# mengcaopku/DCNet

Hardware: AMD Instinct MI355X
Metric: clips/sec (T=8, 416x416, bs8) fwd+bwd (higher is better)
Workload: dtype f32; 1 GPU; T=8 416x416 bs8/GPU L=20 fp32, 64 img/GPU/step as pairs, fwd+5 losses+bwd+RMSprop; arith=f16x2-split MFMA, fp32 accumulate, parallelism=dp1, ranks_seen=1, reducer=none, step=hipGraph replay (fwd+losses+bwd+RMSprop), sampler=mt

## Files before the change

### dcnet_amd/csrc/coattn.hip

```cpp
#include "igemm.h"
#include "prof.h"
#include "coattn.h"

int tn_gemm_batched(const float* A, int lda, long long a_bs, const float* B, int ldb, long long b_bs,
                    float* C, int ldc, long long c_bs, const float* row_scale,
                    int M, int m_ld, int N, int K, int batch, int accumulate, hipStream_t stream,
                    const unsigned* amax_a = nullptr, const unsigned* amax_b = nullptr);

namespace {

constexpr int EXP_ROWS = 32;

typedef _Float16 f16x4c_t __attribute__((ext_vector_type(4)));
constexpr float E_SPLIT_SCALE = 8192.f;
template <bool SPLIT>
__global__ __launch_bounds__(256) void exp_sums_kernel(float* __restrict__ E, int hw, int ldE, float t,
                                                       float* __restrict__ rsum, float* __restrict__ colpart) {
  __shared__ float red[4][EXP_ROWS];
  const int b = blockIdx.y, rb = blockIdx.x;
  const int i0 = rb * EXP_ROWS;
  float* e = E + ((size_t)b * hw + i0) * ldE;
  float racc[EXP_ROWS];
#pragma unroll
  for (int r = 0; r < EXP_ROWS; ++r) racc[r] = 0.f;
  const int nrow = min(EXP_ROWS, hw - i0);
  for (int j = threadIdx.x * 4; j < ldE; j += 1024) {
    f32x4 v[EXP_ROWS];
#pragma unroll
    for (int r = 0; r < EXP_ROWS; ++r)
      v[r] = r < nrow ? *reinterpret_cast<const f32x4*>(e + (size_t)r * ldE + j) : f32x4{0.f, 0.f, 0.f, 0.f};
    f32x4 cs = {0.f, 0.f, 0.f, 0.f};
#pragma unroll
    for (int r = 0; r < EXP_ROWS; ++r) {
      if (r < nrow) {
        f32x4 o;
#pragma unroll
        for (int k = 0; k < 4; ++k) o[k] = (j + k < hw) ? expf(t * v[r][k] - t) : 0.f;
        if constexpr (SPLIT) {
          const f32x4 ts = o * E_SPLIT_SCALE;
          const f16x4c_t h = {(_Float16)ts[0], (_Float16)ts[1], (_Float16)ts[2], (_Float16)ts[3]};
          const f16x4c_t l = {(_Float16)(ts[0] - (float)h[0]), (_Float16)(ts[1] - (float)h[1]), (_Float16)(ts[2] - (float)h[2]),
                              (_Float16)(ts[3] - (float)h[3])};
          unsigned char* run = reinterpret_cast<unsigned char*>(e + (size_t)r * ldE + (j & ~7)) + (j & 4) * 2;
          *reinterpret_cast<f16x4c_t*>(run) = h;
          *reinterpret_cast<f16x4c_t*>(run + 16) = l;
        } else {
          *reinterpret_cast<f32x4*>(e + (size_t)r * ldE + j) = o;
        }
        cs += o; racc[r] += (o[0] + o[1]) + (o[2] + o[3]);
      }
    }
    *reinterpret_cast<f32x4*>(colpart + ((size_t)rb * gridDim.y + b) * ldE + j) = cs;
  }
  const int lane = threadIdx.x & 63, wave = threadIdx.x >> 6;
#pragma unroll
  for (int r = 0; r < EXP_ROWS; ++r) {
    const float s = wave_sum(racc[r]);
    if (lane == 0) red[wave][r] = s;
  }
  __syncthreads();
  if (threadIdx.x < EXP_ROWS && i0 + threadIdx.x < hw)
    rsum[(size_t)b * hw + i0 + threadIdx.x] = 1.f / (red[0][threadIdx.x] + red[1][threadIdx.x] + red[2][threadIdx.x] + red[3][threadIdx.x]);
}

__global__ __launch_bounds__(256) void colsum_inv_kernel(const float* __restrict__ colpart, int nrb, int b, int hw, int ldE,
                                                         float* __restrict__ cinv) {
  const int j = blockIdx.x * 256 + threadIdx.x, bb = blockIdx.y;
  if (j >= hw) return;
  float s = 0.f;
  for (int rb = 0; rb < nrb; ++rb) s += colpart[((size_t)rb * b + bb) * ldE + j];
  cinv[(size_t)bb * hw + j] = 1.f / s;
}

enum { AM_ONE = 0, AM_DO1, AM_DO2, AM_DO1S, AM_DO2S, AM_DA, AM_DP1, AM_DP2, AM_SLOTS };
__global__ __launch_bounds__(256) void amax_init_kernel(unsigned* __restrict__ w) {
  for (int i = threadIdx.x; i < AM_SLOTS * DCN_AMAX_WORDS; i += 256) w[i] = i < DCN_AMAX_WORDS ? 0x3F800000u : 0u;
}

__global__ __launch_bounds__(256) void rowdot_scale_kernel(const float* __restrict__ d, int ldd, int64_t bsd,
                                                           const float* __restrict__ o, int ldo, int64_t bso, int hw,
                                                           const float* __restrict__ inv, int64_t rows, int c,
                                                           float* __restrict__ delta, float* __restrict__ ds,
                                                           unsigned* __restrict__ amax_d, unsigned* __restrict__ amax_ds) {
  __shared__ float red[4];
  const int lane = threadIdx.x & 63;
  const int64_t row = (int64_t)blockIdx.x * 4 + (threadIdx.x >> 6);
  float vmax = 0.f, s = 0.f;
  if (row < rows) {
    const int64_t bb = row / hw, i = row - bb * hw;
    s = inv[row];
    float acc = 0.f;
    for (int k = lane * 4; k < c; k += 256) {
      const f32x4 dv = *reinterpret_cast<const f32x4*>(d + bb * bsd + i * ldd + k);
      const f32x4 ov = *reinterpret_cast<const f32x4*>(o + bb * bso + i * ldo + k);
      acc += dv[0] * ov[0] + dv[1] * ov[1] + dv[2] * ov[2] + dv[3] * ov[3];
      *reinterpret_cast<f32x4*>(ds + row * c + k) = dv * s;
      vmax = fmaxf(fmaxf(vmax, fmaxf(fabsf(dv[0]), fabsf(dv[1]))), fmaxf(fabsf(dv[2]), fabsf(dv[3])));
    }
    acc = wave_sum(acc);
    if (lane == 0) delta[row] = acc;
  }
  const float vs = wave_max(vmax * s);
  amax_update_block(amax_d, vmax, red);
  __syncthreads();
  amax_update_block(amax_ds, vs, red);
}

template <bool ESPLIT, bool OSPLIT = false>
__global__ __launch_bounds__(256) void dA_kernel(const float* __restrict__ E, float* __restrict__ dP1, const float* __restrict__ dP2,
                                                 const float* __restrict__ rinv, const float* __restrict__ cinv,
                                                 const float* __restrict__ d1, const float* __restrict__ d2,
                                                 int hw, int ldE, float t, int64_t total4, unsigned* __restrict__ amax_da) {
  __shared__ float red[4];
  float vmax = 0.f;
  const int l4 = ldE >> 2;
  float s_out = 1.f;
  if constexpr (OSPLIT) {
    const int be = (int)((amax_read(amax_da) >> 23) & 0xFF);
    int ex = (be == 0 || be == 255) ? 0 : 14 - (be - 126);
    ex = ex > 100 ? 100 : (ex < -100 ? -100 : ex);
    s_out = __uint_as_float((unsigned)(ex + 127) << 23);
  }
  for (int64_t idx = (int64_t)blockIdx.x * 256 + threadIdx.x; idx < total4; idx += (int64_t)gridDim.x * 256) {
    const int64_t row = idx / l4;
    const int j = (int)(idx - row * l4) * 4;
    const int64_t bb = row / hw;
    f32x4 e;
    if constexpr (ESPLIT) {
      const unsigned char* run = reinterpret_cast<const unsigned char*>(E + row * ldE + (j & ~7)) + (j & 4) * 2;
      const f16x4c_t h = *reinterpret_cast<const f16x4c_t*>(run), l = *reinterpret_cast<const f16x4c_t*>(run + 16);
#pragma unroll
      for (int k = 0; k < 4; ++k) e[k] = ((float)h[k] + (float)l[k]) * (1.f / E_SPLIT_SCALE);
    } else {
      e = *reinterpret_cast<const f32x4*>(E + row * ldE + j);
    }
    const f32x4 p1 = *reinterpret_cast<const f32x4*>(dP1 + row * ldE + j);
    const f32x4 p2 = *reinterpret_cast<const f32x4*>(dP2 + row * ldE + j);
    const float ri = rinv[row], di = d1[row];
    f32x4 o;
#pragma unroll
    for (int k = 0; k < 4; ++k) {
      float v = 0.f;
      if (j + k < hw) v = t * e[k] * ((p1[k] - di) * ri + (p2[k] - d2[bb * hw + j + k]) * cinv[bb * hw + j + k]);
      o[k] = v;
    }
    if constexpr (OSPLIT) {
      const f32x4 ts = o * s_out;
      const f16x4c_t h = {(_Float16)ts[0], (_Float16)ts[1], (_Float16)ts[2], (_Float16)ts[3]};
      const f16x4c_t l = {(_Float16)(ts[0] - (float)h[0]), (_Float16)(ts[1] - (float)h[1]), (_Float16)(ts[2] - (float)h[2]),
                          (_Float16)(ts[3] - (float)h[3])};
      unsigned char* run = reinterpret_cast<unsigned char*>(dP1 + row * ldE + (j & ~7)) + (j & 4) * 2;
      *reinterpret_cast<f16x4c_t*>(run) = h;
      *reinterpret_cast<f16x4c_t*>(run + 16) = l;
    } else {
      *reinterpret_cast<f32x4*>(dP1 + row * ldE + j) = o;
      vmax = fmaxf(fmaxf(vmax, fmaxf(fabsf(o[0]), fabsf(o[1]))), fmaxf(fabsf(o[2]), fabsf(o[3])));
    }
  }
  if constexpr (!OSPLIT) amax_update_block(amax_da, vmax, red);
}

__global__ __launch_bounds__(64) void da_bound_kernel(const unsigned* __restrict__ a1, const unsigned* __restrict__ a2, float t,
                                                      unsigned* __restrict__ out) {
  const float b = 2.f * t * (__uint_as_float(amax_read(a1)) + __uint_as_float(amax_read(a2)));
  out[threadIdx.x & (DCN_AMAX_WORDS - 1)] = __float_as_uint(b);
}

inline int ld_pad(int hw) { return (hw + 31) / 32 * 32; }

void gemm_params(IgemmParams& p, const float* A, int lda, long long a_bs, const float* B, int ldb, long long b_bs,
                 float* C, int ldc, long long c_bs, int M, int N, int K, int batch) {
  p = IgemmParams{};
  p.osy = p.osx = p.isy = p.isx = 1; p.dense_out = 1;
  p.in = A; p.ldi = lda; p.in_bs = a_bs; p.wt = B; p.ldw = ldb; p.wt_bs = b_bs; p.out = C; p.ldo = ldc; p.out_bs = c_bs;
  p.ldr = ldc;
  p.N = 1; p.Hi = 1; p.Wi = M; p.Ho = 1; p.Wo = M; p.Hs = 1; p.Ws = M; p.M = M;
  p.Ci = K; p.Co = N; p.ntaps = 1; p.batch = batch;
}

}

static bool on_gemm3(int b, int hw, int c) { return c % 32 == 0 && gemm3_applicable(hw, c, hw, b) && gemm3_applicable(hw, hw, c, b); }

int coattn_ld_pad(int hw) { return ld_pad(hw); }
bool coattn_on_gemm3(int b, int hw, int c) { return on_gemm3(b, hw, c); }
unsigned* coattn_ws_amax(float* ws, int b, int hw) { return reinterpret_cast<unsigned*>(ws + (int64_t)cdiv(hw, EXP_ROWS) * b * ld_pad(hw)); }
int coattn_amax_init(unsigned* am, hipStream_t stream) {
  hipLaunchKernelGGL(amax_init_kernel, dim3(1), dim3(256), 0, stream, am);
  DCN_CHECK_LAUNCH("coattn amax_init");
  return DCN_OK;
}
int coattn_exp_sums(float* E, int b, int hw, float temperature, float* rinv, float* cinv, float* ws, bool split, hipStream_t stream) {
  const int ldE = ld_pad(hw), nrb = cdiv(hw, EXP_ROWS);
  const int pid = prof_begin(12, (double)b * hw * ldE * 8.0, stream);
  if (split) hipLaunchKernelGGL(exp_sums_kernel<true>, dim3(nrb, b), dim3(256), 0, stream, E, hw, ldE, temperature, rinv, ws);
  else hipLaunchKernelGGL(exp_sums_kernel<false>, dim3(nrb, b), dim3(256), 0, stream, E, hw, ldE, temperature, rinv, ws);
  prof_end(pid, stream);
  DCN_CHECK_LAUNCH("exp_sums");
  hipLaunchKernelGGL(colsum_inv_kernel, dim3(cdiv(hw, 256), b), dim3(256), 0, stream, ws, nrb, b, hw, ldE, cinv);
  DCN_CHECK_LAUNCH("colsum_inv");
  return DCN_OK;
}

extern "C" int64_t dcn_coattn_fwd_ws(int b, int hw, int c) {
  (void)c;
  return (int64_t)cdiv(hw, EXP_ROWS) * b * ld_pad(hw) + AM_SLOTS * DCN_AMAX_WORDS;
}
extern "C" int64_t dcn_coattn_e_size(int b, int hw) { return (int64_t)b * hw * ld_pad(hw); }
extern "C" int64_t dcn_coattn_saved_size(int b, int hw, int c) {
  return dcn_coattn_e_size(b, hw) + (on_gemm3(b, hw, c) ? (int64_t)2 * b * hw * c : 0);
}

extern "C" int dcn_coattn_fwd(const float* f1, const float* f2, int ldf, int64_t bsf, float* f1_attn, float* f2_attn, int ldo,
                              int64_t bso, float* E, float* rinv, float* cinv, float* ws,
                              int b, int hw, int c, float temperature, void* stream_) {
  hipStream_t stream = (hipStream_t)stream_;
  DCN_CHECK_ARG(f1 && f2 && f1_attn && E && rinv && cinv && ws, "coattn_fwd: null pointer");
  DCN_CHECK_ARG(b > 0 && hw > 0 && c > 0 && c % 32 == 0, "coattn_fwd: bad shape (c=%d must be a multiple of 32)", c);
  if (ldf <= 0) ldf = c;
  if (ldo <= 0) ldo = c;
  DCN_CHECK_ARG(ldf % 4 == 0 && ldo % 4 == 0, "coattn_fwd: ldf/ldo must be multiples of 4");
  if (bsf <= 0) bsf = (int64_t)hw * ldf;
  if (bso <= 0) bso = (int64_t)hw * ldo;
  DCN_CHECK_ARG(bsf % 4 == 0 && bso % 4 == 0, "coattn_fwd: batch strides must be multiples of 4");
  const int ldE = ld_pad(hw);
  unsigned* am = reinterpret_cast<unsigned*>(ws + (int64_t)cdiv(hw, EXP_ROWS) * b * ldE);
  hipLaunchKernelGGL(amax_init_kernel, dim3(1), dim3(256), 0, stream, am);
  DCN_CHECK_LAUNCH("coattn amax_init");
  const unsigned* one = am + AM_ONE * DCN_AMAX_WORDS;
  const int nrb = cdiv(hw, EXP_ROWS);
  const long long bsE = (long long)hw * ldE;
  if (on_gemm3(b, hw, c)) {
    float* f1s = E + dcn_coattn_e_size(b, hw);
    float* f2s = f1s + (int64_t)b * hw * c;
    const long long bss = (long long)hw * c;
    int rc = gemm3_presplit(f1, ldf, bsf, f1s, c, bss, b, hw, c, one, stream);
    if (rc) return rc;
    if ((rc = gemm3_presplit(f2, ldf, bsf, f2s, c, bss, b, hw, c, one, stream))) return rc;
    if ((rc = gemm3_launch(f1s, c, bss, 0, f2s, c, bss, 0, E, ldE, bsE, nullptr, 0, hw, hw, c, b, 0, one, one, stream))) return rc;
    const int pid = prof_begin(12, (double)b * hw * ldE * 8.0, stream);
    hipLaunchKernelGGL(exp_sums_kernel<true>, dim3(nrb, b), dim3(256), 0, stream, E, hw, ldE, temperature, rinv, ws);
    prof_end(pid, stream);
    DCN_CHECK_LAUNCH("exp_sums");
    hipLaunchKernelGGL(colsum_inv_kernel, dim3(cdiv(hw, 256), b), dim3(256), 0, stream, ws, nrb, b, hw, ldE, cinv);
    DCN_CHECK_LAUNCH("colsum_inv");
    if ((rc = gemm3_launch(E, ldE, bsE, 0, f2s, c, bss, 1, f1_attn, ldo, bso, rinv, hw, hw, c, hw, b, 0, one, one, stream))) return rc;
    if (f2_attn) rc = gemm3_launch(E, ldE, bsE, 1, f1s, c, bss, 1, f2_attn, ldo, bso, cinv, hw, hw, c, hw, b, 0, one, one, stream);
    return rc;
  }
  IgemmParams p;
  gemm_params(p, f1, ldf, bsf, f2, ldf, bsf, E, ldE, (long long)hw * ldE, hw, hw, c, b);
  p.amax_a = one; p.amax_b = one;
  int rc = igemm_launch(p, stream);
  if (rc) return rc;
  const int pid = prof_begin(12, (double)b * hw * ldE * 8.0, stream);
  hipLaunchKernelGGL(exp_sums_kernel<false>, dim3(nrb, b), dim3(256), 0, stream, E, hw, ldE, temperature, rinv, ws);
  prof_end(pid, stream);
  DCN_CHECK_LAUNCH("exp_sums");
  hipLaunchKernelGGL(colsum_inv_kernel, dim3(cdiv(hw, 256), b), dim3(256), 0, stream, ws, nrb, b, hw, ldE, cinv);
  DCN_CHECK_LAUNCH("colsum_inv");
  gemm_params(p, E, ldE, (long long)hw * ldE, f2, ldf, bsf, f1_attn, ldo, bso, hw, c, ldE, b);
  p.bmode = 1; p.kvalid = hw; p.row_scale = rinv; p.amax_a = one; p.amax_b = one;
  rc = igemm_launch(p, stream);
  if (rc) return rc;
  if (f2_attn)
    rc = tn_gemm_batched(E, ldE, (long long)hw * ldE, f1, ldf, bsf, f2_attn, ldo, bso,
                         cinv, hw, ldE, c, hw, b, 0, stream, one, one);
  return rc;
}

extern "C" int64_t dcn_coattn_bwd_ws(int b, int hw, int c) {
  return (int64_t)2 * b * hw * ld_pad(hw) + (int64_t)2 * b * hw * c + (int64_t)2 * b * hw + AM_SLOTS * DCN_AMAX_WORDS +
         (on_gemm3(b, hw, c) ? (int64_t)2 * b * hw * c + 4 : 0);
}

extern "C" int dcn_coattn_bwd(const float* f1, const float* f2, int ldf, int64_t bsf,
                              const float* d_f1_attn, const float* d_f2_attn, int lddo, int64_t bsdo,
                              const float* f1_attn, const float* f2_attn, int ldo, int64_t bso,
                              const float* E, const float* rinv, const float* cinv,
                              float* d_f1, float* d_f2, int lddf, int64_t bsdf, int accumulate, float* ws,
                              int b, int hw, int c, float temperature, void* stream_) {
  hipStream_t stream = (hipStream_t)stream_;
  DCN_CHECK_ARG(f1 && f2 && d_f1_attn && d_f2_attn && f1_attn && f2_attn && E && rinv && cinv && d_f1 && d_f2 && ws,
                "coattn_bwd: null pointer");
  DCN_CHECK_ARG(b > 0 && hw > 0 && c > 0 && c % 32 == 0, "coattn_bwd: bad shape");
  if (ldf <= 0) ldf = c;
  if (ldo <= 0) ldo = c;
  if (lddo <= 0) lddo = c;
  if (lddf <= 0) lddf = c;
  if (bsf <= 0) bsf = (int64_t)hw * ldf;
  if (bso <= 0) bso = (int64_t)hw * ldo;
  if (bsdo <= 0) bsdo = (int64_t)hw * lddo;
  if (bsdf <= 0) bsdf = (int64_t)hw * lddf;
  const int ldE = ld_pad(hw);
  const long long rows = (long long)b * hw;
  float* dP1 = ws;
  float* dP2 = dP1 + rows * ldE;
  float* dO1s = dP2 + rows * ldE;
  float* dO2s = dO1s + rows * c;
  float* del1 = dO2s + rows * c;
  float* del2 = del1 + rows;
  unsigned* am = reinterpret_cast<unsigned*>(del2 + rows);
  hipLaunchKernelGGL(amax_init_kernel, dim3(1), dim3(256), 0, stream, am);
  DCN_CHECK_LAUNCH("coattn amax_init");
  auto slot = [&](int i) { return am + i * DCN_AMAX_WORDS; };
  hipLaunchKernelGGL(rowdot_scale_kernel, dim3(cdiv(rows, 4)), dim3(256), 0, stream, d_f1_attn, lddo, bsdo, f1_attn, ldo, bso, hw, rinv, rows, c, del1, dO1s,
                     slot(AM_DO1), slot(AM_DO1S));
  DCN_CHECK_LAUNCH("rowdot_scale");
  hipLaunchKernelGGL(rowdot_scale_kernel, dim3(cdiv(rows, 4)), dim3(256), 0, stream, d_f2_attn, lddo, bsdo, f2_attn, ldo, bso, hw, cinv, rows, c, del2, dO2s,
                     slot(AM_DO2), slot(AM_DO2S));
  DCN_CHECK_LAUNCH("rowdot_scale");
  const int64_t total4 = rows * (ldE / 4);
  int64_t g = (total4 + 255) / 256; if (g > 8192) g = 8192;
  if (g > 1024) g = 1024;
  const long long bsE = (long long)hw * ldE;
  if (on_gemm3(b, hw, c)) {
    float* dO1p = reinterpret_cast<float*>(((uintptr_t)(am + AM_SLOTS * DCN_AMAX_WORDS) + 15) & ~(uintptr_t)15);
    float* dO2p = dO1p + rows * c;
    const float* f1s = E + dcn_coattn_e_size(b, hw);
    const float* f2s = f1s + rows * c;
    const long long bss = (long long)hw * c;
    int rc;
    if ((rc = gemm3_presplit(d_f1_attn, lddo, bsdo, dO1p, c, bss, b, hw, c, slot(AM_DO1), stream))) return rc;
    if ((rc = gemm3_presplit(d_f2_attn, lddo, bsdo, dO2p, c, bss, b, hw, c, slot(AM_DO2), stream))) return rc;
    if ((rc = gemm3_presplit(dO1s, c, bss, dO1s, c, bss, b, hw, c, slot(AM_DO1S), stream))) return rc;
    if ((rc = gemm3_presplit(dO2s, c, bss, dO2s, c, bss, b, hw, c, slot(AM_DO2S), stream))) return rc;
    if ((rc = gemm3_launch(dO1p, c, bss, 0, f2s, c, bss, 0, dP1, ldE, bsE, nullptr, 0, hw, hw, c, b, 0, slot(AM_DO1), slot(AM_ONE), stream, slot(AM_DP1)))) return rc;
    if ((rc = gemm3_launch(f1s, c, bss, 0, dO2p, c, bss, 0, dP2, ldE, bsE, nullptr, 0, hw, hw, c, b, 0, slot(AM_ONE), slot(AM_DO2), stream, slot(AM_DP2)))) return rc;
    hipLaunchKernelGGL(da_bound_kernel, dim3(1), dim3(64), 0, stream, slot(AM_DP1), slot(AM_DP2), temperature, slot(AM_DA));
    DCN_CHECK_LAUNCH("dA bound");
    const int pid_da = prof_begin(31, (double)total4 * 16.0 * 4.0, stream);
    hipLaunchKernelGGL((dA_kernel<true, true>), dim3((int)g), dim3(256), 0, stream, E, dP1, dP2, rinv, cinv, del1, del2, hw, ldE, temperature, total4, slot(AM_DA));
    prof_end(pid_da, stream);
    DCN_CHECK_LAUNCH("dA");
    if ((rc = gemm3_launch(dP1, ldE, bsE, 0, f2s, c, bss, 1, d_f1, lddf, bsdf, nullptr, 0, hw, c, hw, b, accumulate, slot(AM_DA), slot(AM_ONE), stream))) return rc;
    if ((rc = gemm3_launch(E, ldE, bsE, 0, dO2s, c, bss, 1, d_f1, lddf, bsdf, nullptr, 0, hw, c, hw, b, 1, slot(AM_ONE), slot(AM_DO2S), stream))) return rc;
    if ((rc = gemm3_launch(dP1, ldE, bsE, 1, f1s, c, bss, 1, d_f2, lddf, bsdf, nullptr, 0, hw, c, hw, b, accumulate, slot(AM_DA), slot(AM_ONE), stream))) return rc;
    return gemm3_launch(E, ldE, bsE, 1, dO1s, c, bss, 1, d_f2, lddf, bsdf, nullptr, 0, hw, c, hw, b, 1, slot(AM_ONE), slot(AM_DO1S), stream);
  }
  IgemmParams p;
  int rc;
  gemm_params(p, d_f1_attn, lddo, bsdo, f2, ldf, bsf, dP1, ldE, (long long)hw * ldE, hw, hw, c, b);
  p.amax_a = slot(AM_DO1); p.amax_b = slot(AM_ONE);
  if ((rc = igemm_launch(p, stream))) return rc;
  gemm_params(p, f1, ldf, bsf, d_f2_attn, lddo, bsdo, dP2, ldE, (long long)hw * ldE, hw, hw, c, b);
  p.amax_a = slot(AM_ONE); p.amax_b = slot(AM_DO2);
  if ((rc = igemm_launch(p, stream))) return rc;
  const int pid_da = prof_begin(31, (double)total4 * 16.0 * 4.0, stream);
  hipLaunchKernelGGL(dA_kernel<false>, dim3((int)g), dim3(256), 0, stream, E, dP1, dP2, rinv, cinv, del1, del2, hw, ldE, temperature, total4, slot(AM_DA));
  prof_end(pid_da, stream);
  DCN_CHECK_LAUNCH("dA");
  gemm_params(p, dP1, ldE, (long long)hw * ldE, f2, ldf, bsf, d_f1, lddf, bsdf, hw, c, ldE, b);
  p.bmode = 1; p.kvalid = hw; p.accumulate = accumulate; p.amax_a = slot(AM_DA); p.amax_b = slot(AM_ONE);
  if ((rc = igemm_launch(p, stream))) return rc;
  gemm_params(p, E, ldE, (long long)hw * ldE, dO2s, c, (long long)hw * c, d_f1, lddf, bsdf, hw, c, ldE, b);
  p.bmode = 1; p.kvalid = hw; p.accumulate = 1; p.amax_a = slot(AM_ONE); p.amax_b = slot(AM_DO2S);
  if ((rc = igemm_launch(p, stream))) return rc;
  rc = tn_gemm_batched(dP1, ldE, (long long)hw * ldE, f1, ldf, bsf, d_f2, lddf, bsdf,
                       nullptr, hw, ldE, c, hw, b, accumulate, stream, slot(AM_DA), slot(AM_ONE));
  if (rc) return rc;
  return tn_gemm_batched(E, ldE, (long long)hw * ldE, dO1s, c, (long long)hw * c, d_f2, lddf, bsdf,
                         nullptr, hw, ldE, c, hw, b, 1, stream, slot(AM_ONE), slot(AM_DO1S));
}
```

### dcnet_amd/csrc/gemm3.hip

```cpp
#include "igemm.h"
#include "prof.h"

namespace {

typedef _Float16 f16x8_t __attribute__((ext_vector_type(8)));
typedef short s16x4 __attribute__((ext_vector_type(4)));
typedef short s16x8 __attribute__((ext_vector_type(8)));
typedef __attribute__((address_space(3))) void lds_void;

#ifndef G3_ABL
#define G3_ABL 0
#endif
constexpr unsigned G3_OOB = 0x80000000u;
constexpr int G3_BM = 256, G3_BN = 256, G3_STAGES = 4;
constexpr int G3_TILE = 256 * 64;
constexpr int G3_STAGE = 2 * G3_TILE;
constexpr int G3_LDS = G3_STAGES * G3_STAGE;

__device__ __forceinline__ float g3_pow2_scale(unsigned amax_bits) {
  const int be = (int)((amax_bits >> 23) & 0xFF);
  if (be == 0 || be == 255) return 1.f;
  int e = 14 - (be - 126);
  e = e > 100 ? 100 : (e < -100 ? -100 : e);
  return __uint_as_float((unsigned)(e + 127) << 23);
}

struct G3Params {
  const float* A; const float* B; float* C;
  long long a_bs, b_bs, c_bs;
  int lda, ldb, ldc;
  int M, N, K;
  int a_rows, b_rows;
  int a_cols, b_cols;
  int tiles_m, tiles_n;
  const float* row_scale; long long rs_bs;
  int accumulate;
  const unsigned* amax_a; const unsigned* amax_b;
  unsigned* amax_out;
  int var;
  int abl;
};

__device__ __forceinline__ int g3_tswz(int krow) { return (krow & 1) | ((krow & 2) << 1); }

template <bool AT, bool BT, bool H1 = false>
__global__ __launch_bounds__(512, 1) void gemm3_kernel(const G3Params p) {
  extern __shared__ __attribute__((aligned(1024))) unsigned char smem3g[];
  const int tid = threadIdx.x, lane = tid & 63;
  const int wave = __builtin_amdgcn_readfirstlane(tid >> 6);
  const int wm = wave >> 2, wn = wave & 3;
  const int per_batch = p.tiles_m * p.tiles_n;
  const int lin = xcd_remap(blockIdx.x, gridDim.x);
  const int batch = __builtin_amdgcn_readfirstlane(lin / per_batch), t_ = lin - batch * per_batch;
  const int bm = __builtin_amdgcn_readfirstlane(t_ / p.tiles_n), bn = t_ - bm * p.tiles_n;
  const int m0 = bm * G3_BM, n0 = bn * G3_BN;
  const int kslices = (p.K + 15) >> 4;

  const float* a_base = p.A + batch * p.a_bs + (AT ? 0 : (long long)m0 * p.lda);
  const float* b_base = p.B + batch * p.b_bs + (BT ? 0 : (long long)n0 * p.ldb);
  const int a_rows_left = AT ? p.a_rows : p.a_rows - m0, b_rows_left = BT ? p.b_rows : p.b_rows - n0;
  const long long a_bytes = ((long long)(a_rows_left - 1) * p.lda + p.a_cols) * 4, b_bytes = ((long long)(b_rows_left - 1) * p.ldb + p.b_cols) * 4;
  const __amdgpu_buffer_rsrc_t a_rs = __builtin_amdgcn_make_buffer_rsrc((void*)a_base, 0, a_bytes > 0x7FFFFFF0LL ? 0x7FFFFFF0 : (int)a_bytes, 0x00020000);
  const __amdgpu_buffer_rsrc_t b_rs = __builtin_amdgcn_make_buffer_rsrc((void*)b_base, 0, b_bytes > 0x7FFFFFF0LL ? 0x7FFFFFF0 : (int)b_bytes, 0x00020000);

  unsigned voff[4];
  int sstep_a, sstep_b;
#pragma unroll
  for (int e = 0; e < 2; ++e) {
    const int j = 2 * wave + e;
    if (AT) {
      voff[e] = (unsigned)((long long)j * p.lda * 4 + m0 * 4 + ((lane ^ g3_tswz(j)) << 4));
      if (m0 + ((lane ^ g3_tswz(j)) << 2) >= p.a_cols) voff[e] = G3_OOB;
    } else {
      const int row = 16 * j + (lane >> 2), c = (lane & 3) ^ ((row >> 2) & 3);
      voff[e] = row < a_rows_left ? (unsigned)((long long)row * p.lda * 4 + c * 16) : G3_OOB;
    }
    if (BT) {
      voff[2 + e] = (unsigned)((long long)j * p.ldb * 4 + n0 * 4 + ((lane ^ g3_tswz(j)) << 4));
      if (n0 + ((lane ^ g3_tswz(j)) << 2) >= p.b_cols) voff[2 + e] = G3_OOB;
    } else {
      const int row = 16 * j + (lane >> 2), c = (lane & 3) ^ ((row >> 2) & 3);
      voff[2 + e] = row < b_rows_left ? (unsigned)((long long)row * p.ldb * 4 + c * 16) : G3_OOB;
    }
  }
  sstep_a = AT ? 16 * p.lda * 4 : 64;
  sstep_b = BT ? 16 * p.ldb * 4 : 64;
  const int my_dst = 2 * wave * 1024;

  int k_done = 0;
  auto issue_a = [&]() {
    const bool live = k_done < kslices && !(G3_ABL && (p.abl & 1));
    unsigned char* st = smem3g + (k_done & (G3_STAGES - 1)) * G3_STAGE + my_dst;
    int sa_ = live ? k_done * sstep_a : 0;
    if (G3_ABL && (p.abl & 8)) sa_ = 0;
#pragma unroll
    for (int e = 0; e < 2; ++e)
      __builtin_amdgcn_raw_ptr_buffer_load_lds(a_rs, (lds_void*)(st + e * 1024), 16, (int)(live ? voff[e] : G3_OOB), sa_, 0, 0);
  };
  auto issue_b = [&]() {
    const bool live = k_done < kslices && !(G3_ABL && (p.abl & 1));
    unsigned char* st = smem3g + (k_done & (G3_STAGES - 1)) * G3_STAGE + my_dst;
    int sb_ = live ? k_done * sstep_b : 0;
    if (G3_ABL && (p.abl & 8)) sb_ = 0;
#pragma unroll
    for (int e = 0; e < 2; ++e)
      __builtin_amdgcn_raw_ptr_buffer_load_lds(b_rs, (lds_void*)(st + G3_TILE + e * 1024), 16, (int)(live ? voff[2 + e] : G3_OOB), sb_, 0, 0);
    ++k_done;
  };
  auto issue = [&]() { issue_a(); issue_b(); };

  const int g = lane >> 5;
  const int hh = lane >> 5, gg = (lane >> 4) & 1, qq = (lane & 15) >> 2, pp = lane & 3;
  int a_rd[4][2], b_rd[2][2];
#pragma unroll
  for (int mi = 0; mi < 4; ++mi) {
    if (AT) {
      const int c = wm * 128 + mi * 32 + 16 * gg + 4 * pp;
#pragma unroll
      for (int r2 = 0; r2 < 2; ++r2) {
        const int kr = 8 * hh + 4 * r2 + qq;
        a_rd[mi][r2] = kr * 1024 + ((((c >> 3) * 2) ^ g3_tswz(kr)) << 4) + (c & 7) * 2;
      }
    } else {
      const int ar = wm * 128 + mi * 32 + (lane & 31);
      a_rd[mi][0] = ar * 64 + (((2 * g) ^ ((ar >> 2) & 3)) << 4);
      a_rd[mi][1] = ar * 64 + (((2 * g + 1) ^ ((ar >> 2) & 3)) << 4);
    }
  }
#pragma unroll
  for (int ni = 0; ni < 2; ++ni) {
    if (BT) {
      const int c = wn * 64 + ni * 32 + 16 * gg + 4 * pp;
#pragma unroll
      for (int r2 = 0; r2 < 2; ++r2) {
        const int kr = 8 * hh + 4 * r2 + qq;
        b_rd[ni][r2] = G3_TILE + kr * 1024 + ((((c >> 3) * 2) ^ g3_tswz(kr)) << 4) + (c & 7) * 2;
      }
    } else {
      const int br = wn * 64 + ni * 32 + (lane & 31);
      b_rd[ni][0] = G3_TILE + br * 64 + (((2 * g) ^ ((br >> 2) & 3)) << 4);
      b_rd[ni][1] = G3_TILE + br * 64 + (((2 * g + 1) ^ ((br >> 2) & 3)) << 4);
    }
  }
  auto tr_read = [&](const unsigned char* ptr) {
    return __builtin_amdgcn_ds_read_tr16_b64_v4i16((__attribute__((address_space(3))) s16x4*)(ptr));
  };
  auto tfrag = [&](const unsigned char* st, int off0, int off1, int plane) {
    const s16x4 lo = tr_read(st + (off0 ^ (plane << 4))), hi = tr_read(st + (off1 ^ (plane << 4)));
    const s16x8 v = {lo[0], lo[1], lo[2], lo[3], hi[0], hi[1], hi[2], hi[3]};
    return __builtin_bit_cast(f16x8_t, v);
  };

  f32x16 acc[4][2];
#pragma unroll
  for (int mi = 0; mi < 4; ++mi)
#pragma unroll
    for (int ni = 0; ni < 2; ++ni)
#pragma unroll
      for (int r = 0; r < 16; ++r) acc[mi][ni][r] = 0.f;

  for (int s = 0; s < G3_STAGES - 1; ++s) issue();

  asm volatile("s_waitcnt vmcnt(%0)" :: "n"((G3_STAGES - 2) * 4) : "memory");
  if (wm == 1) __builtin_amdgcn_s_barrier();
  for (int it = 0; it < kslices; ++it) {
    __builtin_amdgcn_s_barrier();
    asm volatile("" ::: "memory");
    const unsigned char* st = smem3g + (it & (G3_STAGES - 1)) * G3_STAGE;
    f16x8_t bh[2], bl[2];
    f16x8_t ah[4], al[4];
    if (G3_ABL && (p.abl & 2)) {
#pragma unroll
      for (int ni = 0; ni < 2; ++ni) { bh[ni] = f16x8_t{(_Float16)it, 0, 0, 0, 0, 0, 0, 0}; bl[ni] = bh[ni]; }
#pragma unroll
      for (int mi = 0; mi < 4; ++mi) { ah[mi] = bh[0]; al[mi] = bh[1]; }
    } else {
#pragma unroll
      for (int ni = 0; ni < 2; ++ni) {
        if (BT) { bh[ni] = tfrag(st, b_rd[ni][0], b_rd[ni][1], 0); if constexpr (!H1) bl[ni] = tfrag(st, b_rd[ni][0], b_rd[ni][1], 1); }
        else { bh[ni] = *reinterpret_cast<const f16x8_t*>(st + b_rd[ni][0]); if constexpr (!H1) bl[ni] = *reinterpret_cast<const f16x8_t*>(st + b_rd[ni][1]); }
      }
#pragma unroll
      for (int mi = 0; mi < 4; ++mi) {
        if (AT) { ah[mi] = tfrag(st, a_rd[mi][0], a_rd[mi][1], 0); if constexpr (!H1) al[mi] = tfrag(st, a_rd[mi][0], a_rd[mi][1], 1); }
        else { ah[mi] = *reinterpret_cast<const f16x8_t*>(st + a_rd[mi][0]); if constexpr (!H1) al[mi] = *reinterpret_cast<const f16x8_t*>(st + a_rd[mi][1]); }
      }
    }
    if (p.var >= 1) {
      issue_a();
      if (wm == 1) asm volatile("s_waitcnt vmcnt(%0)" :: "n"((G3_STAGES - 2) * 4 - 2) : "memory");
    } else {
      issue();
      if (wm == 1) asm volatile("s_waitcnt vmcnt(%0)" :: "n"((G3_STAGES - 2) * 4) : "memory");
    }
    asm volatile("s_waitcnt lgkmcnt(0)" ::: "memory");
    __builtin_amdgcn_s_barrier();
    asm volatile("" ::: "memory");
    if (G3_ABL && (p.abl & 4)) {
#pragma unroll
      for (int mi = 0; mi < 4; ++mi) { asm volatile("" :: "v"(ah[mi]), "v"(al[mi])); }
#pragma unroll
      for (int ni = 0; ni < 2; ++ni) { asm volatile("" :: "v"(bh[ni]), "v"(bl[ni])); }
    } else {
      __builtin_amdgcn_s_setprio(1);
      if constexpr (!H1) {
#pragma unroll
        for (int mi = 0; mi < 4; ++mi)
#pragma unroll
          for (int ni = 0; ni < 2; ++ni) acc[mi][ni] = __builtin_amdgcn_mfma_f32_32x32x16_f16(al[mi], bh[ni], acc[mi][ni], 0, 0, 0);
        if (p.var == 2) issue_b();
#pragma unroll
        for (int mi = 0; mi < 4; ++mi)
#pragma unroll
          for (int ni = 0; ni < 2; ++ni) acc[mi][ni] = __builtin_amdgcn_mfma_f32_32x32x16_f16(ah[mi], bl[ni], acc[mi][ni], 0, 0, 0);
      } else if (p.var == 2) issue_b();
#pragma unroll
      for (int mi = 0; mi < 4; ++mi)
#pragma unroll
        for (int ni = 0; ni < 2; ++ni) acc[mi][ni] = __builtin_amdgcn_mfma_f32_32x32x16_f16(ah[mi], bh[ni], acc[mi][ni], 0, 0, 0);
      __builtin_amdgcn_s_setprio(0);
    }
    if (p.var == 1) issue_b();
    if (wm == 0) asm volatile("s_waitcnt vmcnt(%0)" :: "n"((G3_STAGES - 2) * 4) : "memory");
  }
  if (wm == 0) __builtin_amdgcn_s_barrier();
  asm volatile("s_waitcnt vmcnt(0)" ::: "memory");

  const float dq = 1.f / (g3_pow2_scale(amax_read(p.amax_a)) * g3_pow2_scale(amax_read(p.amax_b)));
  float* __restrict__ cb = p.C + batch * p.c_bs;
  const float* rs = p.row_scale ? p.row_scale + batch * p.rs_bs : nullptr;
  float vmax = 0.f;
#pragma unroll
  for (int mi = 0; mi < 4; ++mi)
#pragma unroll
    for (int r = 0; r < 16; ++r) {
      const int m = m0 + wm * 128 + mi * 32 + 4 * g + (r & 3) + 8 * (r >> 2);
      if (m >= p.M) continue;
      const float f = rs ? dq * rs[m] : dq;
#pragma unroll
      for (int ni = 0; ni < 2; ++ni) {
        const int n = n0 + wn * 64 + ni * 32 + (lane & 31);
        if (n >= p.N) continue;
        float v = acc[mi][ni][r] * f;
        float* dst = cb + (long long)m * p.ldc + n;
        if (p.accumulate) v += *dst;
        *dst = v;
        vmax = fmaxf(vmax, fabsf(v));
      }
    }
  if (p.amax_out) {
    vmax = wave_max(vmax);
    if (lane == 0) amax_update(p.amax_out, vmax, blockIdx.x * 8 + wave);
  }
}

__global__ __launch_bounds__(256) void presplit_kernel(const float* __restrict__ src, int ld, long long bs, float* __restrict__ dst, int ldd,
                                                        long long bsd, int rows, int c, long long total8, const unsigned* __restrict__ amax) {
  const float s = g3_pow2_scale(amax_read(amax));
  const int c8 = c >> 3;
  for (long long i = (long long)blockIdx.x * 256 + threadIdx.x; i < total8; i += (long long)gridDim.x * 256) {
    const long long row_all = i / c8; const int o = (int)(i - row_all * c8);
    const long long b = row_all / rows; const int row = (int)(row_all - b * rows);
    const float* sp = src + b * bs + (long long)row * ld + o * 8;
    const f32x4 x0 = *reinterpret_cast<const f32x4*>(sp) * s, x1 = *reinterpret_cast<const f32x4*>(sp + 4) * s;
    f16x8_t h, l;
#pragma unroll
    for (int e = 0; e < 4; ++e) { h[e] = (_Float16)x0[e]; h[4 + e] = (_Float16)x1[e]; }
#pragma unroll
    for (int e = 0; e < 4; ++e) { l[e] = (_Float16)(x0[e] - (float)h[e]); l[4 + e] = (_Float16)(x1[e] - (float)h[4 + e]); }
    float* dp = dst + b * bsd + (long long)row * ldd + o * 8;
    *reinterpret_cast<f16x8_t*>(dp) = h;
    *reinterpret_cast<f16x8_t*>(dp + 4) = l;
  }
}

DCN_KNOB(g_gemm3, "Gemm3", 1, "gemm3.hip: the co-attention products on pre-split operands (0 = implicit-GEMM / weight-gradient tiles; + 256 * v = schedule variant v; + 16 * bits = timing ablations, results WRONG)",
         nullptr, "-DG3_ABL=1", G3_ABL != 0, [](int v) { return (v & 0xF0) != 0; });
DCN_KNOB(g_gemm3_h1, "H1gemm3", 1, "gemm3.hip: one f16 piece per operand in the bf16 precision modes (0 = both pieces, fp32-accurate co-attention)");

template <bool AT, bool BT, bool H1>
int launch3g_(const G3Params& p, int grid, hipStream_t stream) {
  static DcnPerDeviceFlag attr_once;
  if (attr_once.first()) {
    (void)hipFuncSetAttribute(reinterpret_cast<const void*>(&gemm3_kernel<AT, BT, H1>), hipFuncAttributeMaxDynamicSharedMemorySize, G3_LDS);
  }
  hipLaunchKernelGGL((gemm3_kernel<AT, BT, H1>), dim3(grid), dim3(512), G3_LDS, stream, p);
  return DCN_OK;
}
template <bool AT, bool BT>
int launch3g(const G3Params& p, int grid, hipStream_t stream) {
  if (g_gemm3_h1 && igemm_precision() == 2) return launch3g_<AT, BT, true>(p, grid, stream);
  return launch3g_<AT, BT, false>(p, grid, stream);
}

}

int gemm3_variant() { const int v = g_gemm3 >> 8; return (v == 1 || v == 2) ? v : 0; }
extern "C" int dcn_gemm3_variant() { return gemm3_variant(); }

bool gemm3_applicable(int M, int N, int K, int batch) {
  return g_gemm3 && (igemm_precision() == 4 || igemm_precision() == 2) && M >= 512 && N >= 256 && K >= 64 && batch >= 1;
}

int gemm3_presplit(const float* src, int ld, long long bs, float* dst, int ldd, long long bsd, int batch, int rows, int c,
                   const unsigned* amax, hipStream_t stream) {
  DCN_CHECK_ARG(src && dst && amax && c % 8 == 0 && ld % 4 == 0 && ldd % 4 == 0 && bs % 4 == 0 && bsd % 4 == 0, "gemm3_presplit: bad argument");
  const long long total8 = (long long)batch * rows * (c / 8);
  long long g = (total8 + 255) / 256; if (g > 16384) g = 16384;
  hipLaunchKernelGGL(presplit_kernel, dim3((int)g), dim3(256), 0, stream, src, ld, bs, dst, ldd, bsd, rows, c, total8, amax);
  DCN_CHECK_LAUNCH("gemm3_presplit");
  return DCN_OK;
}

int gemm3_launch(const float* A, int lda, long long a_bs, int at, const float* B, int ldb, long long b_bs, int bt,
                 float* C, int ldc, long long c_bs, const float* row_scale, long long rs_bs,
                 int M, int N, int K, int batch, int accumulate, const unsigned* amax_a, const unsigned* amax_b, hipStream_t stream,
                 unsigned* amax_out) {
  DCN_CHECK_ARG(A && B && C && amax_a && amax_b, "gemm3: null pointer");
  DCN_CHECK_ARG(lda % 4 == 0 && ldb % 4 == 0 && a_bs % 4 == 0 && b_bs % 4 == 0 && (((uintptr_t)A | (uintptr_t)B) & 15) == 0, "gemm3: 16-byte rows");
  G3Params p{};
  p.A = A; p.B = B; p.C = C; p.a_bs = a_bs; p.b_bs = b_bs; p.c_bs = c_bs; p.lda = lda; p.ldb = ldb; p.ldc = ldc;
  p.M = M; p.N = N; p.K = K;
  const int k16 = (K + 15) / 16 * 16;
  p.a_rows = at ? K : M; p.b_rows = bt ? K : N;
  p.a_cols = at ? (M + 7) / 8 * 8 : k16; p.b_cols = bt ? (N + 7) / 8 * 8 : k16;
  DCN_CHECK_ARG(p.a_cols <= lda && p.b_cols <= ldb, "gemm3: rows shorter than the tile reads (lda=%d ldb=%d)", lda, ldb);
  p.tiles_m = cdiv(M, G3_BM); p.tiles_n = cdiv(N, G3_BN);
  p.row_scale = row_scale; p.rs_bs = rs_bs; p.accumulate = accumulate; p.amax_a = amax_a; p.amax_b = amax_b; p.amax_out = amax_out; p.abl = (g_gemm3 >> 4) & 15; p.var = gemm3_variant();
  const int grid = p.tiles_m * p.tiles_n * batch;
  const int pid = prof_begin(40, 2.0 * batch * (double)M * N * K, stream);
  int rc;
  if (at) rc = bt ? launch3g<true, true>(p, grid, stream) : DCN_ERR_ARG;
  else rc = bt ? launch3g<false, true>(p, grid, stream) : launch3g<false, false>(p, grid, stream);
  prof_end(pid, stream);
  DCN_CHECK_ARG(rc == DCN_OK, "gemm3: no A^T . B^T form");
  DCN_CHECK_LAUNCH("gemm3");
  return DCN_OK;
}

extern "C" int dcn_gemm3_supported(int m, int n, int k, int batch) { return gemm3_applicable(m, n, k, batch) ? 1 : 0; }

extern "C" int dcn_gemm3_presplit(const float* src, int ld, int64_t bs, float* dst, int ldd, int64_t bsd, int batch, int rows, int c,
                                  const uint32_t* amax, void* stream) {
  return gemm3_presplit(src, ld, bs, dst, ldd, bsd, batch, rows, c, amax, (hipStream_t)stream);
}

extern "C" int dcn_gemm3(const float* a, int lda, int64_t a_bs, int a_t, const float* b, int ldb, int64_t b_bs, int b_t,
                         float* c, int ldc, int64_t c_bs, const float* row_scale, int64_t rs_bs,
                         int m, int n, int k, int batch, int accumulate, const uint32_t* amax_a, const uint32_t* amax_b, void* stream) {
  DCN_CHECK_ARG(m > 0 && n > 0 && k > 0 && batch > 0, "gemm3: empty problem");
  return gemm3_launch(a, lda, a_bs, a_t, b, ldb, b_bs, b_t, c, ldc, c_bs, row_scale, rs_bs, m, n, k, batch, accumulate, amax_a, amax_b,
                      (hipStream_t)stream, nullptr);
}
```

### dcnet_amd/csrc/igemm.h

```cpp
#pragma once
#include "common.h"

#define IGEMM_MAX_TAPS 16


struct IgemmParams {
  const float* in;
  const float* wt;
  const float* f8;
  const unsigned* amax_a;
  const unsigned* amax_b;
  const void* wt16;
  const float* b_scale;
  unsigned* amax_out;
  float* out;
  const float* scale;
  const float* shift;
  const float* residual;
  float* stats;
  const float* row_scale;
  int batch;
  long long in_bs, wt_bs, out_bs;
  int bmode;
  int kvalid;
  int N, Hi, Wi, Ci, ldi;
  int Ho, Wo;
  int Hs, Ws;
  int oy0, ox0, osy, osx;
  int isy, isx;
  int Co, ldo, ldr, ldw;
  int M;
  int ntaps;
  int cpt, kiters;
  int act; float slope;
  int accumulate, dense_out, c4;
  int tap_dy[IGEMM_MAX_TAPS], tap_dx[IGEMM_MAX_TAPS], tap_w[IGEMM_MAX_TAPS];
  int ncls;
  int cls_M[4], cls_Hs[4], cls_Ws[4], cls_oy0[4], cls_ox0[4], cls_ntaps[4];
  const float* bt_y; const float* bt_mean; const float* bt_invstd; const float* bt_gamma; const float* bt_beta;
  int bt_act; float bt_slope;
  const unsigned char* a_scale8; const unsigned char* b_scale8;
};
inline double epilogue_reads(const IgemmParams& p) { return 1.0 + (p.accumulate ? 1.0 : 0.0) + (p.residual ? 1.0 : 0.0) + (p.bt_y ? 1.0 : 0.0); }
bool igemm_tap_capable(const IgemmParams& p);

int igemm_grid_m(int M, int Co, int ntaps);
int igemm_launch(const IgemmParams& p, hipStream_t stream);
bool igemm_will_presplit(long long rows, int Co, int ntaps, int Ci);

bool conv3_applicable(const IgemmParams& p, int precision, int gran);
int conv3_launch(const IgemmParams& p, int gran, hipStream_t stream);
bool conv3x_takes(const IgemmParams& p, int gran);
int conv3x_launch(const IgemmParams& p, int gran, hipStream_t stream);
int conv3b_bm(int M, int Co, int Wi);
bool conv3b_takes(const IgemmParams& p);
int conv3b_launch(const IgemmParams& p, int out_f32, hipStream_t stream);

bool conv1_applicable(const IgemmParams& p, int precision, int gran);
int conv1_launch(const IgemmParams& p, int gran, hipStream_t stream);
int conv1_tile_of(long long rows, int Co, int ntaps, int Ci, int stats, int gran, int storage16);
int conv1b_grid_m(int M, int Co, int ntaps, int s1_w = 0);
int conv1b_launch(const IgemmParams& p, int out_f32, hipStream_t stream);
int conv1q_grid_m(int M, int Co);
int conv1q_launch(const IgemmParams& p, int out_f32, hipStream_t stream);
bool conv2b_takes(int M, int Co, int ntaps);
int conv2b_launch(const IgemmParams& p, int out_f32, hipStream_t stream);


bool stem_applicable(const IgemmParams& p, const float* scratch);
int stem_launch(const IgemmParams& p, float* scratch, hipStream_t stream);

bool dgrad2_applicable(int n, int h, int wd, int cin, int cout, int ksize, int stride, int accumulate);
struct DcnBnTap { const float* y; const float* mean; const float* invstd; const float* gamma; const float* beta; int act; float slope;
                  float* stats; int stats_rows; };
int nconv1_launch_b16(int mode, const void* x, int ldi, const void* w16, void* y, int ldo, float* stats, int stats_rows,
                      int n, int h, int wd, int stride, hipStream_t stream);
int dgrad2_launch_b16(const void* dy, int lddy, const void* wt16, void* dx, int n, int h, int wd, int cin, int accumulate, hipStream_t stream);
int dgrad2_grid(int n, int h, int wd, int cin);
int dgrad2_launch(const float* dy, int lddy, const float* wt, float* dx, int n, int h, int wd, int cin, int accumulate,
                  const uint32_t* amax_dy, const uint32_t* amax_w, const DcnBnTap* tap, hipStream_t stream);
bool gemm3_applicable(int M, int N, int K, int batch);
int gemm3_presplit(const float* src, int ld, long long bs, float* dst, int ldd, long long bsd, int batch, int rows, int c,
                   const unsigned* amax, hipStream_t stream);
int gemm3_launch(const float* A, int lda, long long a_bs, int at, const float* B, int ldb, long long b_bs, int bt,
                 float* C, int ldc, long long c_bs, const float* row_scale, long long rs_bs,
                 int M, int N, int K, int batch, int accumulate, const unsigned* amax_a, const unsigned* amax_b, hipStream_t stream,
                 unsigned* amax_out = nullptr);
int igemm_precision();
extern int g_abl;
extern int g_wsplit;
struct DcnPreAct { const float* scale; const float* shift; int act; float slope; };
bool nconv1_applicable(int mode, int n, int h, int wd, int cin, int cout, int ksize, int stride);
int nconv1_launch(int mode, const float* x, int ldi, const float* w, float* y, int ldo, float* stats, int stats_rows,
                  int n, int h, int wd, int stride, const uint32_t* amax_x, const uint32_t* amax_w, const DcnPreAct* pre, hipStream_t stream);
```

### dcnet_amd/functions.py

```python
from __future__ import annotations

from typing import Optional

import torch

from . import convblock, ops


class ConvBNAct(torch.autograd.Function):

    @staticmethod
    def forward(ctx, x, weight, gamma, beta, bn, ksize: int, training: bool, slope: float, amax_x=None, bank=None, out_b16: bool = False):
        cout = weight.shape[0]
        am = ops.use_amax()
        if bank is not None and x.shape[3] != weight.shape[1]:
            bank = None
        ctx.wparam = convblock.direct_wgrad_param(weight, training)
        ctx.b16 = ops.storage_b16() and bank is not None
        ctx.x_f32 = x.dtype == torch.float32
        w = wsp = aw = ax = ao = None
        if ctx.b16:
            x = ops.to_b16(x.contiguous())
        else:
            if bank is not None:
                w, wsp = bank["ohwi"], bank["split"]
                aw = bank["amax"] if am else None
            else:
                w = ops.weight_to_ohwi(weight, ci_pad=x.shape[3])
                aw = ops.absmax(weight.detach()) if am else None
            ax = (amax_x if amax_x is not None else ops.absmax(x)) if am else None
            ao = ops.amax_slot(x.device) if am else None
        if training:
            y, stats = convblock.conv_forward(x, ksize, 1, cout, w=w, bank=bank, want_stats=True, amax_x=ax, amax_w=aw, w_split=wsp)
            aux, out, _ = convblock.train_bn_forward(y, stats, gamma.detach(), beta.detach(), bn.eps, bn.momentum, bn.running_mean,
                                                     bn.running_var, ops.ACT_LEAKY, slope, bn=bn, amax_out=ao, out_f32=not out_b16)
        else:
            out, aux = convblock.conv_forward(x, ksize, 1, cout, w=w, bank=bank, fold=(gamma.detach(), beta.detach(), bn.running_mean,
                                                                                       bn.running_var, bn.eps),
                                              act=ops.ACT_LEAKY, slope=slope, out_f32=not out_b16, amax_x=ax, amax_w=aw, amax_out=ao, w_split=wsp)
            y = out
        if training or not ctx.b16:
            ctx.save_for_backward(x, y, aux, w, gamma, beta)
        ctx.bank = bank
        ctx.meta = (ksize, training, slope, tuple(weight.shape))
        ctx.amax = (ax, aw)
        if ao is not None:
            ctx.mark_non_differentiable(ao)
        return out, ao

    @staticmethod
    def backward(ctx, dout, _ga=None):
        ksize, training, slope, wshape = ctx.meta
        if ctx.b16 and not training:
            raise NotImplementedError("ConvBNAct, bf16 storage: no backward in eval mode (frozen-BatchNorm fine-tuning is not built)")
        x, y, aux, w, gamma, beta = ctx.saved_tensors
        gamma, beta = gamma.detach(), beta.detach()
        ax, aw = ctx.amax
        bank = ctx.bank
        dout = dout.contiguous()
        ady = None
        if training:
            ady = ops.amax_slot(dout.device) if ops.use_amax() else None
            dy, dgamma, dbeta = ops.bn_act_bwd(y, dout, aux[0], aux[1], gamma, beta, ops.ACT_LEAKY, slope, amax_out=ady,
                                               quant=ctx.needs_input_grad[0] and ops.f8_takes(y.shape[3], x.shape[3], ksize))
        else:
            dy, dgamma, dbeta = convblock.frozen_bn_backward(y, dout, aux[0], gamma, beta, ops.ACT_LEAKY, slope)

        def dgrad():
            if not ctx.needs_input_grad[0]:
                return None
            return convblock.conv_dgrad(dy, x.shape, ksize, 1, w=w, bank=bank, out_f32=ctx.x_f32, amax_dy=ady, amax_w=aw,
                                        wt_ready=bank and (bank["t"], bank["tsplit"]))[0]

        dx, dwt = convblock.schedule_wgrad(x, dy, ksize, 1, wshape, dgrad, amax_x=ax, amax_dy=ady, direct_into=ctx.wparam)
        if ctx.wparam is None:
            ops.join_side(x.device)
        return dx, dwt, dgamma, dbeta, None, None, None, None, None, None, None


class ConvBias(torch.autograd.Function):

    @staticmethod
    def forward(ctx, x, weight, bias, amax_x=None):
        cout = weight.shape[0]
        cop = ops.pad32(cout)
        ctx.wparam = convblock.direct_wgrad_param(weight)
        w = ops.weight_to_ohwi(weight, ci_pad=x.shape[3], co_pad=cop)
        b = torch.zeros(cop, dtype=torch.float32, device=x.device)
        b[:cout] = bias.detach()
        ctx.wshape = tuple(weight.shape)
        ctx.b16 = ops.storage_b16() and weight.shape[2] == 1 and x.shape[3] % 32 == 0
        ctx.x_f32 = x.dtype == torch.float32
        ctx.amax, bank = (None, None), None
        if ctx.b16:
            x = ops.to_b16(x.contiguous())
            w = w.reshape(cop, -1).to(torch.bfloat16)
            bank = {"b16": w.reshape(-1)}
        y, _ = convblock.conv_forward(x, weight.shape[2], 1, cop, w=w, bank=bank, shift=b, out_f32=True)
        ctx.save_for_backward(x, w)
        if not ctx.b16:
            ctx.amax = (amax_x, ops.absmax(weight.detach()) if ops.use_amax() else None)
        return y

    @staticmethod
    def backward(ctx, dy):
        x, w = ctx.saved_tensors
        co, ci, k, _ = ctx.wshape
        ax, aw = ctx.amax
        dy = dy.contiguous()
        rowsum = lambda: ops.colsum_rows(dy.view(-1, dy.shape[-1]))[:co]
        if ctx.b16:
            db = rowsum()
            dy, ady = ops.to_b16(dy), None
        else:
            db = None
            ady = ops.absmax(dy) if ops.use_amax() else None

        def dgrad():
            nonlocal db
            if db is None:
                db = rowsum()
            if not ctx.needs_input_grad[0]:
                return None
            bank = {"tb16": w.t().contiguous().reshape(-1)} if ctx.b16 else None
            return convblock.conv_dgrad(dy, x.shape, k, 1, w=w, bank=bank, out_f32=ctx.x_f32, amax_dy=ady, amax_w=aw)[0]

        dx, dwt = convblock.schedule_wgrad(x, dy, k, 1, ctx.wshape, dgrad, amax_x=ax, amax_dy=ady, after=False, direct_into=ctx.wparam)
        if ctx.wparam is None:
            ops.join_side(x.device)
        return dx, dwt, db, None


class L2Norm(torch.autograd.Function):

    @staticmethod
    def forward(ctx, x):
        out, norm, _, _ = ops.l2norm_score_fwd(x)
        ctx.save_for_backward(out, norm)
        return out

    @staticmethod
    def backward(ctx, dout):
        out, norm = ctx.saved_tensors
        dx, _ = ops.l2norm_score_bwd(out, norm, dout.contiguous(), None, None, 0)
        return dx


class NormScore(torch.autograd.Function):

    @staticmethod
    def forward(ctx, x, q, want_neg: bool):
        n, h, w, e = x.shape
        q = q.contiguous()
        corr, norm, score, flip = ops.l2norm_score_fwd(x, q, h * w, want_flip=want_neg)
        ctx.save_for_backward(corr, norm, q)
        if not want_neg:
            return corr, score.view(n, h, w), None
        return corr, score.view(n, h, w), flip.view(n, h, w)

    @staticmethod
    def backward(ctx, dcorr, dscore, dneg):
        corr, norm, q = ctx.saved_tensors
        q = q.detach()
        n, h, w, _ = corr.shape
        dout = dcorr.contiguous() if dcorr is not None else None
        ds = dscore.contiguous().view(-1) if dscore is not None else None
        dn = dneg.contiguous().view(-1) if dneg is not None else None
        use_q = q if (ds is not None or dn is not None) else None
        dx, dq = ops.l2norm_score_bwd(corr, norm, dout, use_q, ds, h * w, dscore_flip=dn)
        return dx, dq, None


class RowDot(torch.autograd.Function):

    @staticmethod
    def forward(ctx, x, q, flip: bool):
        n, h, w, e = x.shape
        x = x.contiguous(); q = q.contiguous()
        ctx.save_for_backward(x, q)
        ctx.flip = flip
        return ops.rowdot_fwd(x, q, h * w, flip).view(n, h, w)

    @staticmethod
    def backward(ctx, ds):
        x, q = ctx.saved_tensors
        n, h, w, e = x.shape
        dx, dq = ops.rowdot_bwd(x, q.detach(), ds.contiguous().view(-1), h * w, ctx.flip, ctx.needs_input_grad[0], ctx.needs_input_grad[1])
        return dx, dq, None


class NormAccumulate(torch.autograd.Function):

    @staticmethod
    def forward(ctx, x, acc: Optional[torch.Tensor], scale: float):
        out, _, _, _ = ops.l2norm_score_fwd(x, out=acc, out_scale=scale, accumulate=acc is not None)
        ctx.mark_dirty(*([acc] if acc is not None else []))
        return out

    @staticmethod
    def backward(ctx, g):
        raise NotImplementedError("the n_frame (inference) model has no backward; train with pair semantics")


class PhraseAttn(torch.autograd.Function):

    @staticmethod
    def forward(ctx, context, embedded, ids, w0, b0, w1, b1, normalize: bool):
        context = context.contiguous(); embedded = embedded.contiguous(); ids = ids.contiguous()
        d = context.shape[2]
        wa = w0.detach().reshape(-1).contiguous(); wb = None if w1 is None else w1.detach().reshape(-1).contiguous()
        attn, out, vnorm = ops.phrase_attn_fwd(context, embedded, ids, wa, b0.detach(), wb, None if b1 is None else b1.detach(), normalize)
        ctx.save_for_backward(context, embedded, wa, wb if wb is not None else wa.new_empty(0), attn, out,
                              vnorm if vnorm is not None else wa.new_empty(0))
        ctx.meta = (normalize, w1 is not None, tuple(w0.shape), d)
        ctx.mark_non_differentiable(attn)
        return out[0], (out[1] if w1 is not None else None), attn

    @staticmethod
    def backward(ctx, g0, g1, _gattn):
        context, embedded, wa, wb, attn, out, vnorm = ctx.saved_tensors
        normalize, two, wshape, d = ctx.meta
        dout = torch.zeros_like(out) if (g0 is None or (two and g1 is None)) else torch.empty_like(out)
        if g0 is not None:
            ops.copy_slice(g0.contiguous(), dout[0])
        if two and g1 is not None:
            ops.copy_slice(g1.contiguous(), dout[1])
        dctx, demb, dwb = ops.phrase_attn_bwd(context, embedded, wa, wb if two else None, attn, out, vnorm if normalize else None, dout, normalize)
        h = 2 if two else 1
        dw0 = dwb[:d].view(wshape); db0 = dwb[h * d:h * d + 1]
        dw1 = dwb[d:2 * d].view(wshape) if two else None
        db1 = dwb[2 * d + 1:2 * d + 2] if two else None
        return dctx, demb, None, dw0, db0, dw1, db1, None


class HeadTail(torch.autograd.Function):

    @staticmethod
    def forward(ctx, l0, l1, l2, s0, s1, s2, q_loc, coord, w_le, b_le, g_le, be_le, w_lt, b_lt, g_lt, be_lt, bn_le, bn_lt, training: bool):
        logits = [l0.contiguous(), l1.contiguous(), l2.contiguous()]
        B = logits[0].shape[0]
        sims = [s.contiguous().view(B, -1) for s in (s0, s1, s2)]
        P = coord.shape[0]
        cnt = B * P
        det = lambda t: t.detach().contiguous()
        w_le, b_le, g_le, be_le, w_lt, b_lt, g_lt, be_lt = map(det, (w_le, b_le, g_le, be_le, w_lt, b_lt, g_lt, be_lt))
        q_loc = q_loc.contiguous()
        e8, xh, stat, mom = ops.locemb_fwd(coord, w_le, b_le, g_le, be_le, bn_le, training, cnt)
        only, obj_map, objn, X = ops.head_obj(logits, sims, e8)
        wp = ops.pad_rows(w_lt, X.shape[1])
        M = ops.gemm_nt(X, wp).view(B, 8, -1)
        Mp, bp, saved = ops.locbn_fwd(M, mom, b_lt, g_lt, be_lt, bn_lt, training, cnt)
        loc_map = ops.locmod_fwd(e8, Mp, bp, q_loc)
        outbox, loc, mm = ops.head_final_fwd(logits, sims, loc_map)
        if training:
            ops.bump_batches(bn_le); ops.bump_batches(bn_lt)
        ctx.save_for_backward(*logits, *sims, *loc, *only, q_loc, coord, w_le, g_le, be_le, b_lt, g_lt, e8, xh, stat, mom, obj_map, objn, X,
                              wp, M, Mp, bp, saved, mm, bn_lt.running_mean)
        ctx.training = training
        ctx.wshape = tuple(w_lt.shape)
        return (*outbox, *loc, *only)

    @staticmethod
    def backward(ctx, do0, do1, do2, dl0, dl1, dl2, dn0, dn1, dn2):
        sv = ctx.saved_tensors
        logits, sims, loc, only = list(sv[0:3]), list(sv[3:6]), list(sv[6:9]), list(sv[9:12])
        (q_loc, coord, w_le, g_le, be_le, b_lt, g_lt, e8, xh, stat, mom, obj_map, objn, X, wp, M, Mp, bp, saved, mm, rmean_lt) = sv[12:]
        B, P = obj_map.shape
        cnt = B * P
        training = ctx.training
        cg = lambda t: None if t is None else t.contiguous()
        d_out = [cg(do0), cg(do1), cg(do2)]; d_loc = [cg(dl0), cg(dl1), cg(dl2)]; d_only = [cg(dn0), cg(dn1), cg(dn2)]
        dloc_map = ops.head_dloc(logits, sims, loc, d_out, d_loc, mm)
        dE_part, dsum = ops.locmod_bwd(e8, Mp, bp, q_loc, dloc_map)
        dE_a = ops.colsum(dE_part.view(B, P * 8)).view(P, 8)
        dMp = dsum[:, :8]
        dbp = ops.colsum(dsum[:, 8])
        dq_loc = dsum[:, 9]
        dM, gout, dmom = ops.locbn_bwd(M, mom, b_lt, g_lt, rmean_lt, saved, dMp, dbp, training, cnt)
        dM2 = dM.view(B * 8, -1)
        dX = ops.gemm_nn(dM2, wp)
        dwp = ops.gemm_tn(dM2, X)
        dw_lt = ops.pad_rows(dwp, P)
        dobj, dE_b = ops.head_fold(dX, e8, obj_map)
        dlogits, dsim = ops.head_dlogits(logits, sims, loc, only, d_out, d_only, obj_map, objn, dobj)
        g88 = ops.locemb_bwd(coord, w_le, g_le, be_le, xh, stat, dE_a, dE_b, dmom, training)
        shp = [t.shape for t in logits]
        dsim = [d.view(s_[0], s_[1], s_[2]) for d, s_ in zip(dsim, shp)]
        return (*dlogits, *dsim, dq_loc, None, g88[:64].view(8, 8), g88[64:72], g88[72:80], g88[80:88],
                dw_lt.view(ctx.wshape), gout[2], gout[0], gout[1], None, None, None)


class InterframeSample(torch.autograd.Function):

    @staticmethod
    def forward(ctx, fv, raw_neg, top_k: int):
        n, h, w, e = fv.shape
        f = fv.contiguous().view(n, h * w, e)
        index, neg_idx, frame, corr, negf = ops.k9_fwd(f, raw_neg, top_k)
# ... 4 lines not shown

    @staticmethod
    def backward(ctx, d_frame, d_corr, d_neg, _a, _b):
        index, neg_idx = ctx.saved_tensors
        n, h, w, e = ctx.shape
        z = lambda g, like: torch.zeros(like, dtype=torch.float32, device=index.device) if g is None else g.contiguous()
        b, k, m = neg_idx.shape
        dfv = ops.k9_bwd(index, neg_idx, z(d_frame, (b, k, e)), z(d_corr, (b, k, e)), z(d_neg, (b, k, m, e)), h * w)
        return dfv.view(n, h, w, e), None, None


class CrossModalSample(torch.autograd.Function):

    @staticmethod
    def forward(ctx, fv, context, conv_w, conv_b, neg, csr_off, csr_src):
        n, h, w, e = fv.shape
        v = fv.contiguous().view(n, h * w, e)
        context = context.contiguous()
        vit, cn = ops.colnorm_fwd(v)
        lag, ln = ops.lagnorm_fwd(context)
        cols, _ = ops.crossmap(lag, vit, conv_w.detach().contiguous(), conv_b.detach().contiguous())
        lag_pos, neg_cross = ops.k14_gather(lag, vit, cols, neg)
        ctx.save_for_backward(vit, cn, lag, ln, cols, csr_off, csr_src)
        ctx.shape = (n, h, w, e)
        ctx.mark_non_differentiable(cols)
        return vit, lag_pos, neg_cross, cols

    @staticmethod
    def backward(ctx, d_vit, d_lag_pos, d_neg, _c):
        vit, cn, lag, ln, cols, csr_off, csr_src = ctx.saved_tensors
        n, h, w, e = ctx.shape
        hw = h * w
        dq = torch.zeros_like(vit) if d_vit is None else d_vit.contiguous()
        extra = ops.k14_negscatter(d_neg.contiguous(), csr_off, csr_src, hw) if d_neg is not None else None
        dv = ops.colnorm_bwd(vit, cn, dq, extra, n - 1)
        dctx = None
        if d_lag_pos is not None and ctx.needs_input_grad[1]:
            dctx = ops.k14_dlag(lag, ln, cols, d_lag_pos.contiguous())
        return dv.view(n, h, w, e), dctx, None, None, None, None, None


class Contrastive(torch.autograd.Function):

    @staticmethod
    def forward(ctx, q, pos, neg, temperature: float):
        q, pos, neg = q.contiguous(), pos.contiguous(), neg.contiguous()
        ctx.save_for_backward(q, pos, neg)
        ctx.t = temperature
        return ops.contrastive_fwd(q, pos, neg, temperature)

    @staticmethod
    def backward(ctx, g):
        q, pos, neg = ctx.saved_tensors
        dq, dpos, dneg = ops.contrastive_bwd(q, pos, neg, ctx.t, g.contiguous().view(1))
        return dq, dpos, dneg, None


class DenseLosses(torch.autograd.Function):

    @staticmethod
    def forward(ctx, ob0, ob1, ob2, s0, s1, s2, n0, n1, n2, l0, l1, l2, ti, tf, size: int):
        c = lambda t: t.contiguous()
        outbox = [c(ob0), c(ob1), c(ob2)]; sim = [c(s0), c(s1), c(s2)]; neg = [c(n0), c(n1), c(n2)]; loc = [c(l0), c(l1), c(l2)]
        out, lse = ops.dense_loss_fwd(outbox, sim, neg, loc, ti, tf, size)
        ctx.save_for_backward(*outbox, *sim, *neg, *loc, ti, tf, lse)
        ctx.size = size
        return out[0], out[1], out[2]

    @staticmethod
    def backward(ctx, gy, gr, gl):
        sv = ctx.saved_tensors
        outbox, sim, neg, loc = list(sv[0:3]), list(sv[3:6]), list(sv[6:9]), list(sv[9:12])
        ti, tf, lse = sv[12:]
        z = torch.zeros((), dtype=torch.float32, device=ti.device)
        gout = torch.stack([z if g is None else g.reshape(()) for g in (gy, gr, gl)])
        d_ob, d_sim, d_ns, d_loc = ops.dense_loss_bwd(outbox, sim, neg, loc, ti, tf, lse, gout, ctx.size)
        return (*d_ob, *d_sim, *d_ns, *d_loc, None, None, None)


class FusionConvBNAct(torch.autograd.Function):

    @staticmethod
    def forward(ctx, corr, flang, coord, weight, gamma, beta, bn, training: bool, amax_x=None):
        n, h, w, e = corr.shape
        am = ops.use_amax()
        ax = (amax_x if amax_x is not None else ops.absmax(corr)) if am else None
        ao = ops.amax_slot(corr.device) if am else None
        co = weight.shape[0]
        wd = weight.detach().view(co, -1)
        w1 = wd[:, :e].contiguous().view(co, e, 1, 1)
        w2, w3 = wd[:, e:2 * e], wd[:, 2 * e:]
        coord2d = coord.reshape(h * w, -1).contiguous()
        y = ops.fusion_prefill(ops.gemm_nt(flang.detach().contiguous(), w2), coord2d, w3).view(n, h, w, co)
        ctx.b16 = ops.storage_b16() and training and e % 32 == 0 and co % 32 == 0
        aw = bank = None
        if ctx.b16:
            corr = ops.to_b16(corr)
            wk = w1.view(co, e).to(torch.bfloat16)
            bank = {"b16": wk.reshape(-1)}
        else:
            wk = ops.weight_to_ohwi(w1)
            aw = ops.absmax(wk) if am else None
        if training:
            y, stats = convblock.conv_forward(corr, 1, 1, co, w=wk, bank=bank, out=y, want_stats=True, accumulate=True, out_f32=True,
                                              amax_x=ax, amax_w=aw)
            aux, out, _ = convblock.train_bn_forward(y, stats, gamma.detach(), beta.detach(), bn.eps, bn.momentum, bn.running_mean,
                                                     bn.running_var, ops.ACT_LEAKY, 0.0, bn=bn, amax_out=ao, out_b16=ctx.b16)
        else:
            out, aux = convblock.conv_forward(corr, 1, 1, co, w=wk, fold=(gamma.detach(), beta.detach(), bn.running_mean, bn.running_var, bn.eps),
                                              act=ops.ACT_LEAKY, slope=0.0, out=y, accumulate=True, amax_x=ax, amax_w=aw, amax_out=ao)
            y = out
        ctx.save_for_backward(corr, y, aux, wk, gamma, beta, flang, weight)
        ctx.training = training
        ctx.coord2d = coord2d
        ctx.amax = (ax, aw)
        if ao is not None:
            ctx.mark_non_differentiable(ao)
        return out, ao

    @staticmethod
    def backward(ctx, dout, _ga=None):
        corr, y, aux, wk, gamma, beta, flang, weight = ctx.saved_tensors
        gamma, beta = gamma.detach(), beta.detach()
        n, h, w, e = corr.shape
        co = weight.shape[0]
        ax, aw = ctx.amax
        dout = dout.contiguous()
        ady = None
        if ctx.training:
            ady = ops.amax_slot(dout.device) if ops.use_amax() else None
            dy, dgamma, dbeta = ops.bn_act_bwd(y, dout, aux[0], aux[1], gamma, beta, ops.ACT_LEAKY, 0.0, amax_out=ady)
        else:
            dy, dgamma, dbeta = convblock.frozen_bn_backward(y, dout, aux[0], gamma, beta, ops.ACT_LEAKY, 0.0)
        wd = weight.detach().view(co, -1)

        def dgrad():
            if not ctx.needs_input_grad[0]:
                return None
            bank = {"tb16": wk.t().contiguous().reshape(-1)} if ctx.b16 else None
            return convblock.conv_dgrad(dy, corr.shape, 1, 1, w=wk, bank=bank, out_f32=True, amax_dy=ady, amax_w=aw)[0]

        dcorr, dw1 = convblock.schedule_wgrad(corr, dy, 1, 1, (co, e, 1, 1), dgrad, amax_x=ax, amax_dy=ady, after=False)
        ops.join_side(corr.device)
        dweight = torch.empty((co, wd.shape[1]), dtype=torch.float32, device=dy.device)
        d_img = ops.fusion_bwd(ops.to_f32(dy), ctx.coord2d, flang.detach().contiguous(), dweight, e)
        ops.copy_slice(dw1.view(co, e), dweight[:, :e])
        dflang = ops.gemm_nn(d_img, wd[:, e:2 * e]) if ctx.needs_input_grad[1] else None
        return dcorr, dflang, None, dweight.view_as(weight), dgamma, dbeta, None, None, None


class CoAttentionPairs(torch.autograd.Function):

    @staticmethod
    def forward(ctx, fv, temperature: float):
        n, h, w, c = fv.shape
        hw = h * w
        cat = torch.empty((n, hw, 2 * c), dtype=torch.float32, device=fv.device)
        f = fv.view(n, hw, c)
        ops.copy_slice(f, cat[..., :c])
        E, rc = ops.coattn_fwd(f[0::2], f[1::2], cat[0::2, :, c:], cat[1::2, :, c:], temperature)
        out = cat.view(n, h, w, 2 * c)
        ctx.save_for_backward(fv, out, E, rc)
        ctx.temperature = temperature
        return out

    @staticmethod
    def backward(ctx, dcat):
        fv, out, E, rc = ctx.saved_tensors
        n, h, w, c = fv.shape
        hw = h * w
        f, cat = fv.view(n, hw, c), out.view(n, hw, 2 * c)
        dcat = dcat.contiguous().view(n, hw, 2 * c)
        df = torch.empty((n, hw, c), dtype=torch.float32, device=f.device)
        ops.copy_slice(dcat[..., :c], df)
        ops.coattn_bwd(f[0::2], f[1::2], dcat[0::2, :, c:], dcat[1::2, :, c:], cat[0::2, :, c:], cat[1::2, :, c:],
                       E, rc, df[0::2], df[1::2], True, ctx.temperature)
        return df.view(n, h, w, c), None


class CoAttentionCenter(torch.autograd.Function):

    @staticmethod
    def forward(ctx, clips, ctr: int, idx: int, temperature: float):
        b, t, hw, c = clips.shape
        cat = torch.empty((b, hw, 2 * c), dtype=torch.float32, device=clips.device)
        cat[..., :c].copy_(clips[:, ctr])
        ctx.meta = (ctr, idx, temperature)
        if ctx.needs_input_grad[0]:
            o2 = torch.empty((b, hw, 2 * c), dtype=torch.float32, device=clips.device)[..., c:]
            E, rc = ops.coattn_fwd(clips[:, ctr], clips[:, idx], cat[..., c:], o2, temperature)
            ctx.save_for_backward(clips, cat, o2, E, rc)
        else:
            ops.coattn_fwd(clips[:, ctr], clips[:, idx], cat[..., c:], None, temperature)
        return cat

    @staticmethod
    def backward(ctx, g):
        clips, cat, o2, E, rc = ctx.saved_tensors
        ctr, idx, temperature = ctx.meta
        b, t, hw, c = clips.shape
        g = g.contiguous()
        d = torch.zeros_like(clips)
        d[:, ctr].copy_(g[..., :c])
        z2 = torch.zeros((b, hw, 2 * c), dtype=torch.float32, device=g.device)[..., c:]
        ops.coattn_bwd(clips[:, ctr], clips[:, idx], g[..., c:], z2, cat[..., c:], o2, E, rc, d[:, ctr], d[:, idx], True, temperature)
        return d, None, None, None


class ToNCHW(torch.autograd.Function):

    @staticmethod
    def forward(ctx, x, c: int):
        ctx.shape = tuple(x.shape)
        return ops.nhwc_to_nchw(x.contiguous(), c)

    @staticmethod
    def backward(ctx, g):
        n, h, w, ld = ctx.shape
        return ops.nchw_to_nhwc(g.contiguous(), ld), None


class LinearAct(torch.autograd.Function):

    @staticmethod
    def forward(ctx, x, weight, bias, relu: bool):
        x = x.contiguous()
        out = ops.gemm_nt(x, weight.detach(), None if bias is None else bias.detach(), ops.ACT_LEAKY if relu else ops.ACT_NONE)
        ctx.save_for_backward(x, weight, out if relu else x.new_empty(0))
        ctx.relu, ctx.has_bias = relu, bias is not None
        return out

    @staticmethod
    def backward(ctx, dout):
        x, weight, out = ctx.saved_tensors
        dz = dout.contiguous()
        if ctx.relu:
            dz = ops.act_bwd(out, dz, 0.0)
        dx = ops.gemm_nn(dz, weight.detach()) if ctx.needs_input_grad[0] else None
        dw = ops.gemm_tn(dz, x)
        db = ops.colsum(dz) if ctx.has_bias else None
        return dx, dw, db, None


class BatchNormRowsAct(torch.autograd.Function):

    @staticmethod
    def forward(ctx, x, gamma, beta, bn, training: bool, relu: bool):
        x = x.contiguous()
        act = ops.ACT_LEAKY if relu else ops.ACT_NONE
        if training:
            mi = ops.bn_finalize(ops.channel_stats(x), x.shape[0], gamma.detach(), beta.detach(), bn.eps, bn.momentum,
                                 bn.running_mean, bn.running_var)
            ops.bump_batches(bn)
            out = ops.scale_act(x, mi[2], mi[3], act, 0.0)
            ctx.save_for_backward(x, mi, gamma, beta)
        else:
            ss = ops.bn_fold(gamma.detach(), beta.detach(), bn.running_mean, bn.running_var, bn.eps)
            out = ops.scale_act(x, ss[0], ss[1], act, 0.0)
            ctx.save_for_backward(out, ss, gamma, beta)
        ctx.training, ctx.relu = training, relu
        return out

    @staticmethod
    def backward(ctx, dout):
        a, aux, gamma, beta = ctx.saved_tensors
        gamma, beta = gamma.detach(), beta.detach()
        dout = dout.contiguous()
        act = ops.ACT_LEAKY if ctx.relu else ops.ACT_NONE
        if ctx.training:
            dx, dgamma, dbeta = ops.bn_act_bwd(a, dout, aux[0], aux[1], gamma, beta, act, 0.0)
        else:
            dx, dgamma, dbeta = convblock.frozen_bn_backward(a, dout, aux[0], gamma, beta, act, 0.0)
        return dx, dgamma, dbeta, None, None, None


class Embedding(torch.autograd.Function):

    @staticmethod
    def forward(ctx, ids, table):
        ids = ids.contiguous()
        ctx.save_for_backward(ids)
        ctx.vocab = table.shape[0]
        return ops.embedding_fwd(ids, table.detach().contiguous())

    @staticmethod
    def backward(ctx, dout):
        (ids,) = ctx.saved_tensors
        return None, ops.embedding_bwd(ids, dout.contiguous(), ctx.vocab)


class BiLSTM(torch.autograd.Function):

    @staticmethod
    def forward(ctx, x, lengths, *params):
        n, L, I = x.shape
        H = params[1].shape[1]
        x2d = x.contiguous().view(n * L, I)
        det = [p.detach().contiguous() for p in params]
        xg = torch.empty((2, n, L, 4 * H), dtype=torch.float32, device=x.device)
        for d in range(2):
            ops.gemm_nt(x2d, det[4 * d], det[4 * d + 2], out=xg[d].view(n * L, 4 * H))
        lens = lengths.contiguous()
        out, hprev, cprev, acts = ops.bilstm_fwd(xg, det[1], det[5], det[3], det[7], lens)
        ctx.save_for_backward(x2d, lens, acts, hprev, cprev, *params)
        ctx.dims = (n, L, I, H)
        return out

    @staticmethod
    def backward(ctx, dout):
        x2d, lens, acts, hprev, cprev, *params = ctx.saved_tensors
        n, L, I, H = ctx.dims
        det = [p.detach().contiguous() for p in params]
        dxg = ops.bilstm_bwd(dout.contiguous(), det[1], det[5], acts, cprev, lens)
        dx = torch.empty((n * L, I), dtype=torch.float32, device=x2d.device)
        grads = []
        for d in range(2):
            g2 = dxg[d].view(n * L, 4 * H)
            dw_ih = ops.gemm_tn(g2, x2d)
            dw_hh = ops.gemm_tn(g2, hprev[d].view(n * L, H))
            ops.gemm_nn(g2, det[4 * d], out=dx, accumulate=(d == 1))
            db = ops.rows_sum(g2)
            grads += [dw_ih, dw_hh, db, db]
        return (dx.view(n, L, I), None) + tuple(grads)


class LocModule(torch.autograd.Function):

    @staticmethod
    def forward(ctx, E, Mp, bp, q):
        E, Mp, bp, q = E.contiguous(), Mp.contiguous(), bp.contiguous(), q.contiguous()
# ... 9 lines not shown
```

### dcnet_amd/lib.py

```python
from __future__ import annotations

import ctypes
import os
from ctypes import c_char_p, c_double, c_float, c_int, c_int64, c_void_p

_HERE = os.path.dirname(os.path.abspath(__file__))
LIB_PATH = os.path.join(_HERE, "libdcnet_hip.so")

P, I, L, F, D = c_void_p, c_int, c_int64, c_float, c_double

SIGNATURES = {
    "dcn_last_error": (c_char_p, []),
    "dcn_version": (I, []),
    "dcn_nchw_to_nhwc": (I, [P, P, I, I, I, I, I, P]),
    "dcn_nhwc_to_nchw": (I, [P, P, I, I, I, I, I, P]),
    "dcn_oihw_to_ohwi": (I, [P, P, I, I, I, I, I, P]),
    "dcn_ohwi_to_oihw": (I, [P, P, I, I, I, I, I, P]),
    "dcn_conv2d_fwd": (I, [P, P, P, I, I, I, I, I, I, I, P, P, I, F, P, I, I, P, I, P, P, P, P, P, I, P]),
    "dcn_absmax": (I, [P, L, I, I, P, P]),
    "dcn_f8_scale": (I, [P, L, I, I, P, P, P]),
    "dcn_conv2d_stats_rows": (I, [I, I, I, I, I, I]),
    "dcn_conv1_tile": (I, [L, I, I, I, I, I]),
    "dcn_l2norm_score_fwd_form": (I, [I]),
    "dcn_bn_apply_form": (I, [I, I]),
    "dcn_igemm_split_build": (I, [I, I]),
    "dcn_gemm3_variant": (I, []),
    "dcn_conv2d_bwd_data": (I, [P, I, P, P, P, I, I, I, I, I, I, I, I, P, P, P, I, P, P]),
    "dcn_conv2d_bwd_data_tap": (I, [P, I, P, P, P, I, I, I, I, I, I, I, I, P, P, P, I, P, P, P, P, P, P, I, F, P, I, P, P]),
    "dcn_conv2d_bwd_data_tap_rows": (I, [I, I, I, I, I, I, I]),
    "dcn_conv2d_pre_supported": (I, [I, I, I, I, I, I, I]),
    "dcn_conv2d_fwd_pre": (I, [P, P, P, I, I, I, I, I, I, I, P, P, I, F, I, P, P, P, P]),
    "dcn_conv2d_bwd_weight_pre_supported": (I, [I, I, I, I, I, I, I]),
    "dcn_conv2d_bwd_weight_pre": (I, [P, I, P, I, P, P, P, I, I, I, I, I, I, I, P, P, I, F, P, P, P]),
    "dcn_bn_act_amax_bound": (I, [P, P, P, I, F, P, P]),
    "dcn_gemm3_supported": (I, [I, I, I, I]),
    "dcn_gemm3_presplit": (I, [P, I, L, P, I, L, I, I, I, P, P]),
    "dcn_gemm3": (I, [P, I, L, I, P, I, L, I, P, I, L, P, L, I, I, I, I, I, P, P, P]),
    "dcn_filter_job_bytes": (I, []),
    "dcn_prepare_filters": (I, [P, I, I, I, P, L, P]),
    "dcn_conv2d_geom_size": (L, [I, I, I, I, I]),
    "dcn_conv2d_geom": (I, [P, I, I, I, I, I, P]),
    "dcn_conv2d_bwd_weight": (I, [P, I, P, I, P, P, P, P, I, I, I, I, I, I, I, P, P, P]),
    "dcn_conv2d_bwd_weight_ws": (L, [I, I, I, I, I, I, I]),
    "dcn_stem_bwd_weight_bn": (I, [P, P, P, I, P, P, P, P, I, F, P, L, I, I, I, I, P, P, P]),
    "dcn_stem_bwd_weight_bn_ws": (L, [I, I, I]),
    "dcn_stem_bwd_weight_bn_b16": (I, [P, P, P, I, P, P, P, P, I, F, P, L, I, I, I, I, P, P, P]),
    "dcn_bn_ws": (L, [I]),
    "dcn_bn_finalize": (I, [P, I, I, L, P, P, F, F, P, P, P, P, P, P, P, P]),
    "dcn_bn_fold": (I, [P, P, P, P, F, I, P, P, P]),
    "dcn_channel_stats": (I, [P, L, I, I, P, P]),
    "dcn_channel_stats_rows": (I, [L]),
    "dcn_scale_act": (I, [P, P, P, I, F, P, P, L, I, I, P, P]),
    "dcn_bn_act_bwd_reduce": (I, [P, P, I, P, P, P, P, I, F, L, I, P, P]),
    "dcn_bn_bwd_sums": (I, [P, I, I, P, P, P]),
    "dcn_bn_act_bwd_apply": (I, [P, P, I, P, P, P, P, I, F, P, L, L, I, P, P, P]),
    "dcn_act_bwd": (I, [P, P, I, F, L, I, P, P]),
    "dcn_coattn_e_size": (L, [I, I]),
    "dcn_coattn_saved_size": (L, [I, I, I]),
    "dcn_coattn_fwd_ws": (L, [I, I, I]),
    "dcn_coattn_fwd": (I, [P, P, I, L, P, P, I, L, P, P, P, P, I, I, I, F, P]),
    "dcn_coattn_bwd_ws": (L, [I, I, I]),
    "dcn_coattn_bwd": (I, [P, P, I, L, P, P, I, L, P, P, I, L, P, P, P, P, P, I, L, I, P, I, I, I, F, P]),
    "dcn_l2norm_score_fwd": (I, [P, I, P, I, P, P, P, P, L, I, I, F, I, P]),
    "dcn_l2norm_score_bwd": (I, [P, I, P, P, I, P, P, P, P, I, P, L, I, I, P]),
    "dcn_rowdot_fwd": (I, [P, I, P, I, P, L, I, I, P]),
    "dcn_rowdot_bwd": (I, [P, I, P, I, P, P, I, P, L, I, I, P]),
    "dcn_phrase_attn_fwd": (I, [P, P, P, P, P, P, P, P, P, P, I, I, I, I, I, P]),
    "dcn_phrase_attn_bwd_ws": (L, [I, I, I]),
    "dcn_phrase_attn_bwd": (I, [P, P, P, P, P, P, P, P, P, P, P, P, I, I, I, I, I, P]),
    "dcn_colsum": (I, [P, I, I, I, P, P]),
    "dcn_locemb_fwd": (I, [P, P, P, P, P, P, P, F, F, I, L, I, P, P, P, P, P]),
    "dcn_locemb_bwd": (I, [P, P, P, P, P, P, P, P, P, I, I, P, P]),
    "dcn_head_obj": (I, [P, P, P, P, P, P, P, P, P, I, P]),
    "dcn_pad_rows": (I, [P, I, P, I, I, I, I, P]),
    "dcn_locbn_fwd": (I, [P, P, P, P, P, P, P, F, F, I, I, L, I, P, P, P, P]),
    "dcn_locbn_bwd": (I, [P, P, P, P, P, P, P, L, P, I, I, L, I, P, P, P, P]),
    "dcn_head_final_fwd": (I, [P, P, P, P, P, P, P, P, I, P]),
    "dcn_head_dloc": (I, [P, P, P, P, P, P, P, P, P, I, P]),
    "dcn_head_fold": (I, [P, P, P, I, I, I, P, P, P]),
    "dcn_head_dlogits": (I, [P, P, P, P, P, P, P, P, P, P, P, P, P, I, P]),
    "dcn_k9_fwd": (I, [P, P, P, I, I, I, I, I, P, P, P, P, P, P]),
    "dcn_k9_bwd": (I, [P, P, P, P, P, I, I, I, I, I, P, P]),
    "dcn_colnorm_fwd": (I, [P, I, I, I, P, P, P]),
    "dcn_colnorm_bwd": (I, [P, P, P, P, I, I, I, I, P, P]),
    "dcn_lagnorm_fwd": (I, [P, I, I, I, P, P, P]),
    "dcn_crossmap": (I, [P, P, P, P, I, I, I, I, P, P, P]),
    "dcn_k14_gather": (I, [P, P, P, P, I, I, I, I, I, P, P, P]),
    "dcn_k14_negscatter": (I, [P, P, P, I, I, P, P]),
    "dcn_k14_dlag": (I, [P, P, P, P, I, I, I, I, P, P]),
    "dcn_build_target": (I, [P, P, I, I, P, P, P]),
    "dcn_target_dense": (I, [P, P, I, I, P, P, P]),
    "dcn_dense_loss_fwd": (I, [P, P, P, P, P, P, I, I, P, P, P, P]),
    "dcn_dense_loss_bwd": (I, [P, P, P, P, P, P, P, P, I, I, P, P, P, P, P]),
    "dcn_contrastive_fwd": (I, [P, P, P, L, I, I, F, P, P, P]),
    "dcn_contrastive_bwd": (I, [P, P, P, L, I, I, F, P, P, P, P, P]),
    "dcn_decode_boxes": (I, [P, P, I, I, P, P, P]),
    "dcn_box_iou": (I, [P, P, I, P, P]),
    "dcn_gemm_nt_batched": (I, [P, I, L, P, I, L, P, I, L, I, I, I, I, P]),
    "dcn_mt_sample_crossmodal_csr": (I, [P, I, I, I, P, P]),
    "dcn_upsample2_nhwc": (I, [P, I, P, I, I, I, I, I, P]),
    "dcn_upsample2_nhwc_bwd": (I, [P, I, P, I, I, I, I, I, I, P]),
    "dcn_copy_slice": (I, [P, I, P, I, L, I, I, P]),
    "dcn_locmod_fwd": (I, [P, P, P, P, P, I, I, I, P]),
    "dcn_locmod_bwd_ws": (L, [I, I]),
    "dcn_locmod_bwd": (I, [P, P, P, P, P, P, P, P, I, I, I, P]),
    "dcn_gemm_nt": (I, [P, I, P, I, P, I, I, I, I, P, I, P, I, I, P]),
    "dcn_gemm_nn": (I, [P, I, P, I, P, I, I, I, I, I, I, P]),
    "dcn_gemm_tn": (I, [P, I, P, I, P, I, I, I, I, I, P]),
    "dcn_lstm_cell_fwd": (I, [P, P, P, P, I, P, P, P, P, I, I, I, P]),
    "dcn_lstm_cell_bwd": (I, [P, I, P, P, P, P, P, I, P, I, P, P, I, I, P]),
    "dcn_bilstm_sync_bytes": (L, []),
    "dcn_bilstm_fwd": (I, [P, P, P, P, P, P, P, P, P, P, P, I, I, I, P]),
    "dcn_bilstm_bwd": (I, [P, P, P, P, P, P, P, P, I, I, I, P]),
    "dcn_rmsprop_step": (I, [P, P, P, P, I, F, P, F, F, F, P]),
    "dcn_adam_prepare": (I, [P, P, I, F, P, D, D, P]),
    "dcn_adam_step": (I, [P, P, P, P, P, P, I, D, D, F, F, P]),
    "dcn_sgd_step": (I, [P, P, P, P, I, F, P, F, F, P]),
    "dcn_fusion_prefill": (I, [P, P, P, I, P, I, I, I, P]),
    "dcn_fusion_bwd_ws": (L, [I, I]),
    "dcn_fusion_bwd": (I, [P, P, P, P, P, P, P, I, I, I, I, I, P]),
    "dcn_row_lengths": (I, [P, I, I, P, P]),
    "dcn_embedding_fwd": (I, [P, P, P, I, I, I, P]),
    "dcn_embedding_bwd": (I, [P, P, P, I, I, I, P]),
    "dcn_set_tuning": (I, [c_char_p, I]),
    "dcn_tuning_info": (I, [I, P, P, P, P, P]),
    "dcn_stream_create": (P, [I]),
    "dcn_stream_destroy": (I, [P]),
    "dcn_stream_priority_range": (I, [P, P]),
    "dcn_prof_enable": (I, [I]),
    "dcn_prof_collect": (I, [P, P, P, P]),
    "dcn_prof_records": (I, [P, P, P, P, I]),
    "dcn_mt_sample_interframe": (I, [P, P, I, I, I, I, P]),
    "dcn_mt_sample_crossmodal": (I, [P, I, I, I, P]),
    "dcn_quant_job_bytes": (I, []),
    "dcn_quant_rows_e4m3_batched": (I, [P, I, I, L, P]),
    "dcn_mt_sample_step": (I, [P, I, I, I, I, I, P, P, P, P, P]),
    "dcn_device_sample_ws": (L, [I]),
    "dcn_device_sample": (I, [P, I, I, I, I, I, P, P, P, P, P, P]),
    "dcn_conv2d_stats_rows_b16": (I, [I, I, I, I, I, I]),
    "dcn_conv2d_fwd_b16": (I, [P, P, P, I, I, I, I, I, I, I, I, P, P, I, F, P, I, I, P, I, P]),
    "dcn_conv2d_bwd_data_b16": (I, [P, I, P, P, I, I, I, I, I, I, I, I, I, P, P, P, P, P, I, F, P, I, P, P]),
    "dcn_conv2d_bwd_weight_ws_b16": (L, [I, I, I, I, I, I, I]),
    "dcn_conv2d_bwd_weight_b16": (I, [P, I, P, I, P, P, P, P, I, I, I, I, I, I, I, P]),
    "dcn_scale_act_b16": (I, [P, I, P, P, I, F, P, I, P, I, L, I, I, P]),
    "dcn_bn_act_bwd_reduce_rows_b16": (I, [L]),
    "dcn_bn_act_bwd_reduce_b16": (I, [P, I, P, I, I, P, P, P, P, I, F, L, I, P, P]),
    "dcn_bn_act_bwd_apply_b16": (I, [P, I, P, I, I, P, P, P, P, I, F, P, L, L, I, P, P]),
    "dcn_cast_rows": (I, [P, I, I, P, I, I, L, I, I, P]),
    "dcn_upsample2_nhwc_b16": (I, [P, I, P, I, I, I, I, I, P]),
    "dcn_upsample2_nhwc_bwd_b16": (I, [P, I, P, I, I, I, I, I, I, P]),
    "dcn_quant_rows_e4m3": (I, [P, I, L, I, P, I, P, P]),
    "dcn_quant_fusable": (I, [I]),
    "dcn_scale_act_b16_q": (I, [P, P, P, I, F, P, I, P, L, I, P, P, P]),
    "dcn_bn_act_bwd_apply_b16_q": (I, [P, P, I, P, P, P, P, I, F, P, L, L, I, P, P, P, P]),
    "dcn_conv2d_stats_rows_f8": (I, [I, I, I, I, I, I]),
    "dcn_conv2d_fwd_f8": (I, [P, P, P, P, P, I, I, I, I, I, I, I, I, P, P, I, F, P, I, I, P, I, P]),
    "dcn_conv2d_bwd_data_f8": (I, [P, P, P, P, P, I, I, I, I, I, I, I, I, I, P, P, P, P, P, I, F, P, I, P, P]),
    "dcn_post_topk": (I, [P, P, P, P, P, I, I, I, I, P, P, P, P, P, P, P, P, P]),
    "dcn_post_fusion": (I, [P, P, P, P, I, I, I, I, P, P, P]),
    "dcn_clip_prep_ws": (L, [I, I]),
    "dcn_clip_prep": (I, [P, L, P, P, I, I, P, P, P, P]),
    "dcn_bank_write": (I, [P, I, P, P, L, I, P]),
    "dcn_coattn_bank_fwd": (I, [P, P, P, P, L, P, P, I, L, P, P, P, P, I, I, I, F, P]),
    "dcn_post_fusion_bank": (I, [P, P, I, I, I, I, P, P, P]),
}
_VALUE_FUNCS = {"dcn_version", "dcn_conv2d_stats_rows", "dcn_conv2d_bwd_data_tap_rows", "dcn_conv2d_pre_supported",
                "dcn_conv2d_bwd_weight_pre_supported", "dcn_gemm3_supported", "dcn_channel_stats_rows", "dcn_filter_job_bytes", "dcn_prof_records",
                "dcn_conv2d_stats_rows_b16", "dcn_bn_act_bwd_reduce_rows_b16", "dcn_conv2d_stats_rows_f8", "dcn_quant_fusable", "dcn_quant_job_bytes",
                "dcn_conv1_tile", "dcn_l2norm_score_fwd_form", "dcn_bn_apply_form", "dcn_igemm_split_build", "dcn_gemm3_variant"}
ABI_VERSION = 313


class DcnError(RuntimeError):
    pass


class _Lib:
    def __init__(self, path: str):
        if not os.path.exists(path):
            raise DcnError(
                f"{path} not found: build it with `python -m dcnet_amd.build` "
                "(hipcc --offload-arch=gfx950).  There is no CPU or eager fallback.")
        self._dll = ctypes.CDLL(path)
        for name, (res, args) in SIGNATURES.items():
            try:
                fn = getattr(self._dll, name)
            except AttributeError as e:
                raise DcnError(f"{path} does not export {name}; rebuild the library") from e
            fn.restype = res
            fn.argtypes = args
            if res is I and name not in _VALUE_FUNCS:
                setattr(self, name[4:], self._checked(name, fn))
            else:
                setattr(self, name[4:], fn)
        for kv in [t for t in os.environ.get("DCN_TUNE", "").split(",") if t]:
            k_, v_ = kv.split("=")
            if self._dll.dcn_set_tuning(k_.encode(), int(v_)) != 0:
                raise DcnError(f"DCN_TUNE: {self._dll.dcn_last_error().decode()}")
        if self._dll.dcn_version() != ABI_VERSION:
            raise DcnError(f"{path} has ABI version {self._dll.dcn_version()}, this binding was written for {ABI_VERSION}: "
                           "rebuild the library (python -m dcnet_amd.build --force)")

    def _checked(self, name, fn):
        def call(*a):
            rc = fn(*a)
            if rc != 0:
                raise DcnError(f"{name} failed ({rc}): {self._dll.dcn_last_error().decode()}")
        call.__name__ = name
        return call


def tuning(L: "_Lib" = None) -> dict:
    dll = (L or lib())._dll
    out = {}
    name, desc, val, dflt, abl = c_char_p(), c_char_p(), c_int(), c_int(), c_int()
    while dll.dcn_tuning_info(len(out), ctypes.byref(name), ctypes.byref(val), ctypes.byref(dflt), ctypes.byref(desc), ctypes.byref(abl)) == 0:
        out[name.value.decode()] = {"value": val.value, "default": dflt.value, "desc": desc.value.decode(), "ablation": abl.value}
    return out


def ablation_build() -> bool:
    return tuning()["abl"]["ablation"] == 2


_lib = None


def lib() -> _Lib:
    global _lib
    if _lib is None:
        _lib = _Lib(LIB_PATH)
    return _lib
```

### dcnet_amd/model.py

```python
from __future__ import annotations

import os
import ctypes
import random
import threading
import time
from collections import OrderedDict
from typing import List, Optional

import numpy as np
import torch
import torch.nn as nn
import torch.nn.functional as F

from . import convblock, ops
from .darknet import Darknet
from .functions import (BatchNormRowsAct, BiLSTM, CoAttentionCenter, CoAttentionPairs, ConvBias, ConvBNAct, CrossModalSample,
                        Embedding, FusionConvBNAct, HeadTail, InterframeSample, L2Norm, LinearAct, NormAccumulate, NormScore, PhraseAttn, RowDot)
from .lib import lib


class OutputList(list):
    __slots__ = ("stacked", "stream", "neg_sim")

# ... 121 lines not shown
                                    bidirectional=True, input_dropout_p=0.2, variable_lengths=True)
        self.temperature = 10.
        self.sub_attn = PhraseAttention(self.textdim)
        self.loc_embedding = nn.Sequential(nn.Linear(8, 8), nn.BatchNorm1d(8), nn.ReLU())
        self.loc_text_embedding = nn.Sequential(nn.Linear(self.num_pos, self.embdim), nn.BatchNorm1d(self.embdim), nn.ReLU())
        self.loc_attn = PhraseAttention(self.textdim)
        self.mapping_visu = nn.Sequential(OrderedDict([
            ("0", ConvBatchNormReLU(1024, emb_size, 1, 1, 0, 1, leaky=leaky)),
            ("1", ConvBatchNormReLU(512, emb_size, 1, 1, 0, 1, leaky=leaky)),
            ("2", ConvBatchNormReLU(256, emb_size, 1, 1, 0, 1, leaky=leaky))]))
        self.mapping_lang = nn.Sequential(
            nn.Linear(self.textdim, emb_size), nn.BatchNorm1d(emb_size), nn.ReLU(), nn.Dropout(jemb_drop_out),
            nn.Linear(emb_size, emb_size), nn.BatchNorm1d(emb_size), nn.ReLU())
        self.corr_conv = nn.Sequential(OrderedDict([
            (str(i), nn.Sequential(ConvBatchNormReLU(emb_size * 2, emb_size, 1, 1, 0, 1, leaky=leaky))) for i in range(3)]))
        self.feature_map = nn.Sequential(
            nn.Conv1d(in_channels=query_len, out_channels=query_len, stride=1, kernel_size=3, padding=1, bias=True),
            nn.Softmax(dim=1))
        embin_size = emb_size * 2 + 8
        if light:
            self.fcn_emb = nn.Sequential(OrderedDict([
                (str(i), nn.Sequential(ConvBatchNormReLU(embin_size, emb_size, 1, 1, 0, 1, leaky=leaky))) for i in range(3)]))
            self.fcn_out = nn.Sequential(OrderedDict([
                (str(i), nn.Sequential(nn.Conv2d(emb_size, 3 * 5, kernel_size=1))) for i in range(3)]))
        else:
            self.fcn_emb = nn.Sequential(OrderedDict([
                (str(i), nn.Sequential(ConvBatchNormReLU(embin_size, emb_size, 1, 1, 0, 1, leaky=leaky),
                                       ConvBatchNormReLU(emb_size, emb_size, 3, 1, 1, 1, leaky=leaky),
                                       ConvBatchNormReLU(emb_size, emb_size, 1, 1, 0, 1, leaky=leaky))) for i in range(3)]))
            self.fcn_out = nn.Sequential(OrderedDict([
                (str(i), nn.Sequential(ConvBatchNormReLU(emb_size, emb_size // 2, 1, 1, 0, 1, leaky=leaky),
                                       nn.Conv2d(emb_size // 2, 3 * 5, kernel_size=1))) for i in range(3)]))
        self._coord_cache = {}
        self._pinned = {}
        self.sampler_busy_s = 0.0
        self._spec = None
        self.static_samples = None
        self.sampler = "mt"
        self.sampler_seed = 0x5DC0E7A1
        self._dev_sampler = {}
        self._streams = {}
        self.sampling_stream = True
        self.presample_ahead = True
        self.language_stream = True
        self.defer_language_backward = False
        self.last_choices = {}

    def finish_backward(self) -> None:
        st = self.__dict__.pop("_lang_pending", None)
        if st is None:
            return
        side = st["side"]
        main = torch.cuda.current_stream()
        pairs = [(t_, l_.grad) for t_, l_ in zip(st["live"], st["leaves"]) if t_.requires_grad and l_.grad is not None]
        hops = []
        events = list(st["events"].values())
        st["event"] = events[-1] if events else None
        if st["event"] is not None:
            if torch.cuda.is_current_stream_capturing():
                for i_ in range(int(ops.LANGUAGE_BWD_HOPS_B16 if ops.storage_b16() else ops.LANGUAGE_BWD_HOPS)):
                    h_ = self._side_stream(main.device, "hop%d" % i_)
                    h_.wait_event(st["event"])
                    with torch.cuda.stream(h_):
                        self._hop_word(main.device).zero_()
                    hops.append(h_)
            for ev_ in reversed(events):
                side.wait_event(ev_)
        else:
            side.wait_stream(main)
        if pairs:
            with torch.cuda.stream(side):
                for _, g_ in pairs:
                    g_.record_stream(side)
                torch.autograd.backward([t_ for t_, _ in pairs], [g_ for _, g_ in pairs])
        main.wait_stream(side)
        for h_ in hops:
            main.wait_stream(h_)
        for l_ in st["leaves"]:
            l_.grad = None

    def _hop_word(self, device):
        key = ("hop_word", str(device))
        if key not in self._streams:
            self._streams[key] = torch.zeros(1, dtype=torch.int32, device=device)
        return self._streams[key]

    def _side_stream(self, device, name: str = "lang"):
        key = (str(device), name)
        if key not in self._streams:
            self._streams[key] = torch.cuda.Stream(device=device)
        return self._streams[key]

    def _head_filter_banks(self):
        if not ops.FILTER_BANKS or not (ops.use_amax() or ops.storage_b16()):
            for blk in self._head_blocks():
                blk.__dict__["_dcn_bank"] = None
            return
        blocks = self._head_blocks()
        fb = convblock.cached_filter_banks(self.__dict__, "_hbanks", {i: b.conv.weight.detach() for i, b in enumerate(blocks)})
        fb.refresh()
        for i, b in enumerate(blocks):
            b.__dict__["_dcn_bank"] = fb.get(i, b.conv.weight)

    def _head_blocks(self):
        out = []
        for seq in (self.mapping_visu, self.corr_conv, self.fcn_emb, self.fcn_out):
            for m in seq.modules():
                if isinstance(m, ConvBatchNormReLU):
                    out.append(m)
        return out

    def _coord(self, h, w, device):
        key = (h, w, str(device))
        if key not in self._coord_cache:
            self._coord_cache[key] = generate_coord_nhwc(h, w, device)
        return self._coord_cache[key]

    def _language(self, word_id):
        raw_flang, context, embedded = self.textmodel(word_id)
        ml = self.mapping_lang
        z = LinearAct.apply(raw_flang, ml[0].weight, ml[0].bias, False)
        z = BatchNormRowsAct.apply(z, ml[1].weight, ml[1].bias, ml[1], self.training, True)
        z = ml[3](z)
        z = LinearAct.apply(z, ml[4].weight, ml[4].bias, False)
        z = BatchNormRowsAct.apply(z, ml[5].weight, ml[5].bias, ml[5], self.training, True)
        flang = L2Norm.apply(z)
        return word_id, flang, context, embedded

    def _fusion_head(self, s: int, corr, flang):
        h, w = corr.shape[1], corr.shape[2]
        ops.region("fusion")
        blk0 = self.fcn_emb[s][0]
        one = ops.amax_const(corr.device, 1.0) if ops.use_amax() else None
        z, za = FusionConvBNAct.apply(corr.contiguous(), flang, self._coord(h, w, corr.device), blk0.conv.weight,
                                      blk0.bn.weight, blk0.bn.bias, blk0.bn, self.training, one)
        z._dcn_amax = za
        chain = list(self.fcn_emb[s])[1:] + list(self.fcn_out[s])[:-1]
        if ops.storage_b16() and self.training and chain and (not ops.FILTER_BANKS or (self.emb_size // 2) % 32):
            raise RuntimeError("bf16 storage: the head chain fcn_emb -> fcn_out runs on bf16 tensors and needs the prepared filter banks "
                               f"(ops.FILTER_BANKS) and emb_size // 2 a multiple of 32 (emb_size = {self.emb_size})")
        n_emb = len(self.fcn_emb[s]) - 1
        for i_, blk in enumerate(chain):
            if i_ == n_emb:
                ops.region("out")
            blk.__dict__["_dcn_out_b16"] = True
            z = blk(z)
        last = self.fcn_out[s][-1]
        if z.dtype == torch.bfloat16 and not ops.storage_b16():
            z = ops.to_f32(z)
        return ConvBias.apply(z, last.weight, last.bias, getattr(z, "_dcn_amax", None))

    def _scale_pairs(self, s: int, raw_s, flang, flang_attn):
        ops.region("mapping")
        fv = L2Norm.apply(self.mapping_visu[s](raw_s, self.visumodel._tap_amax[s]))
        ops.region("corr")
        one = ops.amax_const(raw_s.device, 1.0) if ops.use_amax() else None
        corr_raw = self.corr_conv[s][0](CoAttentionPairs.apply(fv, self.temperature), one)
        corr, sim, neg_sim = NormScore.apply(corr_raw, flang_attn, self.training)
        return fv, corr, sim, neg_sim, self._fusion_head(s, corr, flang)

    def _map_scale(self, s: int, raw_s):
        return self.mapping_visu[s](raw_s, self.visumodel._tap_amax[s])

    def _corr_accumulate(self, s: int, cat, acc, scale: float):
        one = ops.amax_const(cat.device, 1.0) if ops.use_amax() else None
        return NormAccumulate.apply(self.corr_conv[s][0](cat, one), acc, scale)

    def _score_scale(self, s: int, corr, flang, flang_attn):
        return RowDot.apply(corr, flang_attn, False), self._fusion_head(s, corr, flang)

    def _scale_nframe(self, s: int, raw_s, flang, flang_attn, B: int, n_frame: int):
        one = ops.amax_const(raw_s.device, 1.0) if ops.use_amax() else None
        fv = L2Norm.apply(self._map_scale(s, raw_s))
        _, h, w, e = fv.shape
        clips = fv.view(B, n_frame, h * w, e)
        ctr, acc = n_frame // 2, None
        for idx in range(n_frame):
            if idx == ctr:
                continue
            cat = CoAttentionCenter.apply(clips, ctr, idx, self.temperature).view(B, h, w, 2 * e)
            z = self.corr_conv[s][0](cat, one)
            if torch.is_grad_enabled() and z.requires_grad:
                zn = L2Norm.apply(z)
                acc = zn * (1.0 / (n_frame - 1)) if acc is None else acc + zn * (1.0 / (n_frame - 1))
            else:
                acc = NormAccumulate.apply(z, acc, 1.0 / (n_frame - 1))
        corr = acc
        sim, logits = self._score_scale(s, corr, flang, flang_attn)
        return fv, corr, sim, None, logits

    def _coord_rows(self, grids, device):
        key = ("rows", tuple(grids), str(device))
        if key not in self._coord_cache:
            self._coord_cache[key] = torch.cat([self._coord(g[0], g[1], device).reshape(-1, 8) for g in grids], dim=0).contiguous()
        return self._coord_cache[key]

    def _head(self, sim_score, logits, flang_loc):
        dev = flang_loc.device
        coord = self._coord_rows([(l.shape[1], l.shape[2]) for l in logits], dev)
        le, lt = self.loc_embedding, self.loc_text_embedding
        res = HeadTail.apply(*logits, *sim_score, flang_loc, coord, le[0].weight, le[0].bias, le[1].weight, le[1].bias,
                             lt[0].weight, lt[0].bias, lt[1].weight, lt[1].bias, le[1], lt[1], self.training)
        return list(res[0:3]), list(res[3:6]), list(res[6:9])

    def _presample_start(self, n, g0, top_k=30, neg_n=10, neg_c=5):
        hw = g0 * g0
        if n < 2 or hw - 1 < neg_n or hw - 1 < neg_c or hw * hw < top_k:
            raise ValueError(f"correspondence sampling needs >= 2 images and a coarsest grid of more than {max(neg_n, neg_c)} "
                             f"cells with >= {top_k} cell pairs (got {n} images, {g0}x{g0})")
        key = (n, hw, top_k, neg_n, neg_c)
        if key not in self._pinned:
            mk = lambda: (torch.empty((n // 2, top_k, neg_n), dtype=torch.int64).pin_memory(),
                          torch.empty((n, hw, neg_c), dtype=torch.int64).pin_memory(),
                          torch.empty(hw + 1, dtype=torch.int32).pin_memory(),
                          torch.empty(n * hw * neg_c, dtype=torch.int32).pin_memory())
            self._pinned[key] = {"sets": [mk(), mk()], "events": [None, None], "turn": 0}
        pin = self._pinned[key]
        which = pin["turn"]; pin["turn"] ^= 1
        k9, k14, csr_off, csr_src = pin["sets"][which]
        if pin["events"][which] is not None:
            pin["events"][which].synchronize()
            pin["events"][which] = None
        st, arr = _mt_state()
        L = lib()
        box = {"err": None, "shape": (n, top_k, hw, neg_n, neg_c), "pin": pin, "which": which, "g0": g0}

        secs = ctypes.c_double(0.0)

        def work():
            try:
                L.mt_sample_step(arr.ctypes.data, n, top_k, hw, neg_n, neg_c, k9.data_ptr(), k14.data_ptr(), csr_off.data_ptr(),
                                 csr_src.data_ptr(), ctypes.byref(secs))
            except BaseException as e:
                box["err"] = e
            box["busy_s"] = secs.value

        th = threading.Thread(target=work, daemon=True)
        th.start()
        return th, st, arr, (k9, k14, csr_off, csr_src), box

    def _presample_take(self, n, g0):
        spec, self._spec = self._spec, None
        if spec is not None:
            th, st, arr, bufs, box = spec
            if box["shape"][0] == n and box["g0"] == g0 and random.getstate() == st:
                return spec
            th.join()
        return self._presample_start(n, g0)

    def device_samples(self, n: int, g0: int, device, top_k=30, neg_n=10, neg_c=5) -> dict:
        hw = g0 * g0
        if n < 2 or hw - 1 < neg_n or hw - 1 < neg_c or hw * hw < top_k:
            raise ValueError(f"correspondence sampling needs >= 2 images and a coarsest grid of more than {max(neg_n, neg_c)} "
                             f"cells with >= {top_k} cell pairs (got {n} images, {g0}x{g0})")
        key = (torch.device(device).index, n, hw, top_k, neg_n, neg_c)
        st = self._dev_sampler.get(key)
        if st is None:
            if torch.cuda.is_current_stream_capturing():
                raise RuntimeError("grounding_model.device_samples: first use inside a stream capture (run one eager step first)")
            st = dict(self.sample_buffers(n, device, top_k, neg_n, neg_c, g0=g0))
            st["state"] = torch.tensor([int(self.sampler_seed) & 0x7FFFFFFFFFFFFFFF, 0], dtype=torch.int64, device=device)
            st["ws"] = torch.zeros(int(lib().device_sample_ws(hw)), dtype=torch.int32, device=device)
            self._dev_sampler[key] = st
        lib().device_sample(st["state"].data_ptr(), n, top_k, hw, neg_n, neg_c, st["k9"].data_ptr(), st["k14"].data_ptr(),
                            st["csr_off"].data_ptr(), st["csr_src"].data_ptr(), st["ws"].data_ptr(),
                            torch.cuda.current_stream().cuda_stream)
        return {k_: st[k_] for k_ in ("k9", "k14", "csr_off", "csr_src")}

    def sample_buffers(self, n: int, device, top_k=30, neg_n=10, neg_c=5, g0=None) -> dict:
        hw = (self.img_size // 32 if g0 is None else g0) ** 2
        return {"k9": torch.zeros((n // 2, top_k, neg_n), dtype=torch.int64, device=device),
                "k14": torch.zeros((n, hw, neg_c), dtype=torch.int64, device=device),
                "csr_off": torch.zeros(hw + 1, dtype=torch.int32, device=device),
                "csr_src": torch.zeros(n * hw * neg_c, dtype=torch.int32, device=device)}

    def draw_samples(self, n: int, into: dict) -> dict:
        handle = self._presample_take(n, self.img_size // 32)
        return self._presample_join(handle, into["k9"].device, ahead=self.presample_ahead, into=into)

    def _presample_join(self, handle, device, ahead=False, into=None):
        th, st, arr, (k9, k14, csr_off, csr_src), box = handle
        th.join()
        if box["err"] is not None:
            raise box["err"]
        self.sampler_busy_s += box.get("busy_s", 0.0)
        if random.getstate() != st:
            st, arr = _mt_state()
            n, top_k, hw, neg_n, neg_c = box["shape"]
            L = lib()
            L.mt_sample_interframe(arr.ctypes.data, 0, n // 2, top_k, hw, neg_n, k9.data_ptr())
            L.mt_sample_crossmodal(arr.ctypes.data, n, hw, neg_c, k14.data_ptr())
            L.mt_sample_crossmodal_csr(k14.data_ptr(), n, hw, neg_c, csr_off.data_ptr(), csr_src.data_ptr())
        _mt_restore(st, arr)
        if device is None:
            return None
        if into is not None:
            for k_, src in (("k9", k9), ("k14", k14), ("csr_off", csr_off), ("csr_src", csr_src)):
                into[k_].copy_(src, non_blocking=True)
            out = into
        else:
            out = {"k9": k9.to(device, non_blocking=True), "k14": k14.to(device, non_blocking=True),
                   "csr_off": csr_off.to(device, non_blocking=True), "csr_src": csr_src.to(device, non_blocking=True)}
        ev = torch.cuda.Event(); ev.record()
        box["pin"]["events"][box["which"]] = ev
        if ahead:
            self._spec = self._presample_start(box["shape"][0], box["g0"])
        return out

    def _interframe_sampling(self, fv0, presampled, top_k=30):
        frame, corr, negf, index, neg_idx = InterframeSample.apply(fv0, presampled["k9"], top_k)
# ... 143 lines not shown
```

### dcnet_amd/ops.py

```python
from __future__ import annotations

from typing import Optional, Tuple

import os

import torch

from .lib import DcnError, ablation_build, lib

ACT_NONE, ACT_LEAKY = 0, 1

PRECISIONS = {"fp32_mfma": 0, "fp32_bf16x3": 1, "bf16": 2, "fp8": 3, "fp32": 4, "bf16s": 2, "fp8s": 2}
_precision = "fp32"


def set_precision(mode: str) -> None:
    global _precision
    if mode not in PRECISIONS:
        raise ValueError(f"precision {mode!r}: expected one of {sorted(PRECISIONS)}")
    lib().set_tuning(b"precision", PRECISIONS[mode])
    _precision = mode


def storage_b16() -> bool:
# ... 761 lines not shown
        qs = torch.empty(rows, dtype=torch.uint8, device=y.device)
        if residual is not None:
            _rows16(residual, "scale_act residual")
        lib().scale_act_b16_q(y.data_ptr(), _p(scale), _p(shift), act, float(slope), _p(residual), 0 if residual is None else residual.stride(-2),
                              out.data_ptr(), rows, c, q8.data_ptr(), qs.data_ptr(), _s())
        out._dcn_q8 = (q8, qs)
        return out
    if _b16(y) or out_b16 or _b16(out):
        if out is None:
            out = torch.empty(y.shape, dtype=torch.float32 if out_f32 else torch.bfloat16, device=y.device)
        if not y.is_contiguous() or (residual is not None and not _b16(residual)):
            raise ValueError("scale_act (bf16 storage): contiguous y, bf16 residual")
        _rows16(out, "scale_act out")
        if residual is not None:
            _rows16(residual, "scale_act residual")
        lib().scale_act_b16(y.data_ptr(), int(not _b16(y)), _p(scale), _p(shift), act, float(slope), _p(residual),
                            0 if residual is None else residual.stride(-2), out.data_ptr(), int(not _b16(out)), rows, c, out.stride(-2), _s())
        return out
    if out is None:
        out = torch.empty_like(y)
    _chk(y, "scale_act y"); _rows(out, "scale_act out")
    lib().scale_act(y.data_ptr(), _p(scale), _p(shift), act, float(slope), _p(residual), out.data_ptr(), rows, c,
                    out.stride(-2), _p(amax_out), _s())
    return out


def _bn_bwd_partials(y, dout, mean, invstd, gamma, beta, act, slope, part):
    c = y.shape[-1]
    rows = y.numel() // c
    if part is not None:
        return part, part.shape[0]
    if _b16(dout) or _b16(y):
        r = lib().bn_act_bwd_reduce_rows_b16(rows)
        part = scratch(r * 2 * c, y.device, slot=0)
        lib().bn_act_bwd_reduce_b16(y.data_ptr(), int(not _b16(y)), dout.data_ptr(), int(not _b16(dout)), dout.stride(-2), mean.data_ptr(), invstd.data_ptr(),
                                    _p(gamma), _p(beta), act, float(slope), rows, c, part.data_ptr(), _s())
        return part, r
    r = lib().channel_stats_rows(rows)
    part = scratch(r * 2 * c, y.device, slot=0)
    lib().bn_act_bwd_reduce(y.data_ptr(), dout.data_ptr(), dout.stride(-2), mean.data_ptr(), invstd.data_ptr(), _p(gamma), _p(beta),
                            act, float(slope), rows, c, part.data_ptr(), _s())
    return part, r


def bn_act_bwd(y, dout, mean, invstd, gamma, beta, act, slope, amax_out=None, part=None, quant=False):
    c = y.shape[-1]
    rows = y.numel() // c
    dev = y.device
    lddo = dout.stride(-2)
    part, r = _bn_bwd_partials(y, dout, mean, invstd, gamma, beta, act, slope, part)
    sums = torch.empty((2, c), dtype=torch.float32, device=dev)
    ws = scratch(lib().bn_ws(c), dev, slot=2)
    lib().bn_bwd_sums(part.data_ptr(), r, c, sums.data_ptr(), ws.data_ptr(), _s())
    if _b16(dout) or _b16(y):
        dy = torch.empty(y.shape, dtype=torch.bfloat16, device=dev)
        if quant and _b16(y) and _b16(dout) and lib().quant_fusable(c):
            q8 = torch.empty(y.shape, dtype=torch.uint8, device=dev)
            qs = torch.empty(rows, dtype=torch.uint8, device=dev)
            lib().bn_act_bwd_apply_b16_q(y.data_ptr(), dout.data_ptr(), lddo, mean.data_ptr(), invstd.data_ptr(), _p(gamma), _p(beta), act, float(slope),
                                         sums.data_ptr(), rows, rows, c, dy.data_ptr(), q8.data_ptr(), qs.data_ptr(), _s())
            dy._dcn_q8 = (q8, qs)
            return dy, sums[1], sums[0]
        lib().bn_act_bwd_apply_b16(y.data_ptr(), int(not _b16(y)), dout.data_ptr(), int(not _b16(dout)), lddo, mean.data_ptr(), invstd.data_ptr(), _p(gamma),
                                   _p(beta), act, float(slope), sums.data_ptr(), rows, rows, c, dy.data_ptr(), _s())
        return dy, sums[1], sums[0]
    dy = torch.empty_like(y)
    lib().bn_act_bwd_apply(y.data_ptr(), dout.data_ptr(), lddo, mean.data_ptr(), invstd.data_ptr(), _p(gamma), _p(beta),
                           act, float(slope), sums.data_ptr(), rows, rows, c, dy.data_ptr(), _p(amax_out), _s())
    return dy, sums[1], sums[0]


def stem_bwd_weight_bn(x, y, dout, mean, invstd, gamma, beta, act, slope, part=None):
    n, h, wd, c = y.shape
    rows = n * h * wd
    dev = y.device
    lddo = dout.stride(-2)
    part, r = _bn_bwd_partials(y, dout, mean, invstd, gamma, beta, act, slope, part)
    sums = torch.empty((2, c), dtype=torch.float32, device=dev)
    ws = scratch(lib().bn_ws(c), dev, slot=2)
    lib().bn_bwd_sums(part.data_ptr(), r, c, sums.data_ptr(), ws.data_ptr(), _s())
    dw = torch.empty((c, 64), dtype=torch.float32, device=dev)
    slabs = scratch(lib().stem_bwd_weight_bn_ws(n, h, wd), dev, slot=0)
    fn = lib().stem_bwd_weight_bn_b16 if _b16(dout) else lib().stem_bwd_weight_bn
    fn(x.data_ptr(), y.data_ptr(), dout.data_ptr(), lddo, mean.data_ptr(), invstd.data_ptr(), _p(gamma), _p(beta),
       act, float(slope), sums.data_ptr(), rows, n, h, wd, c, dw.data_ptr(), slabs.data_ptr(), _s())
    return dw, sums[1], sums[0]


_nbt = None


def bump_batches(bn) -> None:
    if _nbt is not None:
        _nbt.append(bn.num_batches_tracked)
    else:
        bn.num_batches_tracked += 1


def batches_begin() -> None:
    global _nbt
    _nbt = []


def batches_end() -> None:
    global _nbt
    pend, _nbt = _nbt, None
    if pend:
        torch._foreach_add_(pend, 1)


LANGUAGE_LATE = True
LANGUAGE_BWD_HOPS = 1
LANGUAGE_BWD_HOPS_B16 = 0
LANGUAGE_BWD_DEFERRED = True
STEM_FUSED_BWD = True
BN_TAP = True
BN_TAP_TRUNK = os.environ.get("DCN_BN_TAP_TRUNK", "1") != "0"


def act_bwd(out, dout, slope):
    c = out.shape[-1]
    rows = out.numel() // c
    dy = torch.empty_like(out)
    lib().act_bwd(out.data_ptr(), dout.data_ptr(), dout.stride(-2), float(slope), rows, c, dy.data_ptr(), _s())
    return dy


def coattn_fwd(f1, f2, out1, out2, temperature):
    b, hw, c = f1.shape
    dev = f1.device
    E = torch.empty(lib().coattn_saved_size(b, hw, c), dtype=torch.float32, device=dev)
    rc = torch.empty((2, b, hw), dtype=torch.float32, device=dev)
    ws = scratch(lib().coattn_fwd_ws(b, hw, c), dev, slot=0)
    assert f1.stride() == f2.stride() and (out2 is None or out1.stride() == out2.stride())
    lib().coattn_fwd(f1.data_ptr(), f2.data_ptr(), f1.stride(1), f1.stride(0), out1.data_ptr(), _p(out2), out1.stride(1),
                     out1.stride(0), E.data_ptr(), rc[0].data_ptr(), rc[1].data_ptr(), ws.data_ptr(), b, hw, c,
                     float(temperature), _s())
    return E, rc


def coattn_bwd(f1, f2, d_out1, d_out2, out1, out2, E, rc, d_f1, d_f2, accumulate, temperature):
    b, hw, c = f1.shape
    ws = scratch(lib().coattn_bwd_ws(b, hw, c), f1.device, slot=0)
    assert f1.stride() == f2.stride() and d_out1.stride() == d_out2.stride() and out1.stride() == out2.stride()
    assert d_f1.stride() == d_f2.stride()
    lib().coattn_bwd(f1.data_ptr(), f2.data_ptr(), f1.stride(1), f1.stride(0),
                     d_out1.data_ptr(), d_out2.data_ptr(), d_out1.stride(1), d_out1.stride(0),
                     out1.data_ptr(), out2.data_ptr(), out1.stride(1), out1.stride(0),
                     E.data_ptr(), rc[0].data_ptr(), rc[1].data_ptr(),
                     d_f1.data_ptr(), d_f2.data_ptr(), d_f1.stride(1), d_f1.stride(0), int(accumulate), ws.data_ptr(),
                     b, hw, c, float(temperature), _s())


def gemm3_presplit(x, amax, out=None):
    b, rows, c = x.shape
    if out is None:
        out = torch.empty((b, rows, c), dtype=torch.float32, device=x.device)
    lib().gemm3_presplit(x.data_ptr(), x.stride(1), x.stride(0), out.data_ptr(), out.stride(1), out.stride(0), b, rows, c, amax.data_ptr(), _s())
    return out


def gemm3(a, b, out, m, n, k, amax_a, amax_b, a_t=False, b_t=False, row_scale=None, accumulate=False):
    lib().gemm3(a.data_ptr(), a.stride(1), a.stride(0), int(a_t), b.data_ptr(), b.stride(1), b.stride(0), int(b_t),
                out.data_ptr(), out.stride(1), out.stride(0), _p(row_scale), 0 if row_scale is None else row_scale.stride(0),
                m, n, k, a.shape[0], int(accumulate), amax_a.data_ptr(), amax_b.data_ptr(), _s())
    return out


def l2norm_score_fwd(x, q=None, rows_per_image=0, out=None, want_flip=False, out_scale=1.0, accumulate=False):
    c = x.shape[-1]
    rows = x.numel() // c
    if out is None:
        out = torch.empty(x.shape, dtype=torch.float32, device=x.device)
    _rows(x, "l2norm x"); _rows(out, "l2norm out")
    norm = torch.empty(rows, dtype=torch.float32, device=x.device)
    score = torch.empty(rows, dtype=torch.float32, device=x.device) if q is not None else None
    flip = torch.empty(rows, dtype=torch.float32, device=x.device) if (q is not None and want_flip) else None
    lib().l2norm_score_fwd(x.data_ptr(), x.stride(-2), out.data_ptr(), out.stride(-2), norm.data_ptr(), _p(q), _p(score), _p(flip),
                           rows, rows_per_image, c, float(out_scale), int(accumulate), _s())
    return out, norm, score, flip


def l2norm_score_bwd(out, norm, dout, q, dscore, rows_per_image, want_dq=True, dscore_flip=None):
    c = out.shape[-1]
    rows = out.numel() // c
    _rows(out, "l2norm_bwd out")
    if dout is not None:
        _rows(dout, "l2norm_bwd dout")
    dx = torch.empty(out.shape, dtype=torch.float32, device=out.device)
    dq = None
    if q is not None and (dscore is not None or dscore_flip is not None) and want_dq:
        dq = torch.empty((rows // rows_per_image, c), dtype=torch.float32, device=out.device)
    lib().l2norm_score_bwd(out.data_ptr(), out.stride(-2), norm.data_ptr(), _p(dout), 0 if dout is None else dout.stride(-2),
                           _p(q), _p(dscore), _p(dscore_flip), dx.data_ptr(), c, _p(dq), rows, rows_per_image, c, _s())
    return dx, dq


def rowdot_fwd(x, q, rows_per_image, flip=False):
    c = x.shape[-1]
    rows = x.numel() // c
    _rows(x, "rowdot x"); _chk(q, "rowdot q")
    score = torch.empty(rows, dtype=torch.float32, device=x.device)
    lib().rowdot_fwd(x.data_ptr(), x.stride(-2), q.data_ptr(), int(flip), score.data_ptr(), rows, rows_per_image, c, _s())
    return score


def rowdot_bwd(x, q, dscore, rows_per_image, flip=False, want_dx=True, want_dq=True):
    c = x.shape[-1]
    rows = x.numel() // c
    dx = torch.empty(x.shape, dtype=torch.float32, device=x.device) if want_dx else None
    dq = torch.empty((rows // rows_per_image, c), dtype=torch.float32, device=x.device) if want_dq else None
    lib().rowdot_bwd(x.data_ptr(), x.stride(-2), q.data_ptr(), int(flip), dscore.data_ptr(), _p(dx), c, _p(dq), rows, rows_per_image, c, _s())
    return dx, dq


def phrase_attn_fwd(context, embedded, ids, w0, b0, w1=None, b1=None, normalize=True):
    n, L, d = context.shape
    e = embedded.shape[2]
    _chk(context, "phrase context"); _chk(embedded, "phrase embedded")
    if not (ids.is_cuda and ids.dtype == torch.int64 and ids.is_contiguous()):
        raise ValueError("phrase_attn: ids must be a contiguous int64 CUDA tensor")
    heads = 1 if w1 is None else 2
    attn = torch.empty((heads, n, L), dtype=torch.float32, device=context.device)
    out = torch.empty((heads, n, e), dtype=torch.float32, device=context.device)
    vnorm = torch.empty((heads, n), dtype=torch.float32, device=context.device) if normalize else None
    lib().phrase_attn_fwd(context.data_ptr(), embedded.data_ptr(), ids.data_ptr(), w0.data_ptr(), b0.data_ptr(), _p(w1), _p(b1),
                          attn.data_ptr(), out.data_ptr(), _p(vnorm), n, L, d, e, int(normalize), _s())
    return attn, out, vnorm


def phrase_attn_bwd(context, embedded, w0, w1, attn, out, vnorm, dout, normalize=True):
    n, L, d = context.shape
    e = embedded.shape[2]
    heads = 1 if w1 is None else 2
    dctx = torch.empty_like(context); demb = torch.empty_like(embedded)
    dwb = torch.empty(heads * d + heads, dtype=torch.float32, device=context.device)
    ws = scratch(lib().phrase_attn_bwd_ws(n, d, heads), context.device, slot=0)
    _chk(dout, "phrase dout")
    lib().phrase_attn_bwd(context.data_ptr(), embedded.data_ptr(), w0.data_ptr(), _p(w1), attn.data_ptr(), out.data_ptr(), _p(vnorm),
                          dout.data_ptr(), dctx.data_ptr(), demb.data_ptr(), dwb.data_ptr(), ws.data_ptr(), n, L, d, e, int(normalize), _s())
    return dctx, demb, dwb


def colsum(x2d):
    if not (x2d.is_cuda and x2d.dtype == torch.float32 and x2d.dim() == 2 and x2d.stride(1) == 1):
        raise ValueError("colsum: expected an fp32 CUDA [rows][cols] view with contiguous columns")
    rows, cols = x2d.shape
    out = torch.empty(cols, dtype=torch.float32, device=x2d.device)
    lib().colsum(x2d.data_ptr(), x2d.stride(0), rows, cols, out.data_ptr(), _s())
    return out


def fusion_prefill(a_img, coord2d, w3):
    n, co = a_img.shape
    hw = coord2d.shape[0]
    _chk(a_img, "fusion_prefill A"); _chk(coord2d, "fusion_prefill coord")
    assert w3.shape == (co, 8) and w3.stride(1) == 1
    out = torch.empty((n, hw, co), dtype=torch.float32, device=a_img.device)
    lib().fusion_prefill(a_img.data_ptr(), coord2d.data_ptr(), w3.data_ptr(), w3.stride(0), out.data_ptr(), n, hw, co, _s())
    return out


def fusion_bwd(dy, coord2d, flang, dweight, e):
    n, co = dy.shape[0], dy.shape[-1]
    hw = dy.numel() // (n * co)
    _chk(dy, "fusion_bwd dy"); _chk(flang, "fusion_bwd flang"); _chk(dweight, "fusion_bwd dweight")
    d_img = torch.empty((n, co), dtype=torch.float32, device=dy.device)
    ws = scratch(lib().fusion_bwd_ws(n, co), dy.device, slot=0)
    ld = dweight.stride(0)
    lib().fusion_bwd(dy.data_ptr(), coord2d.data_ptr(), flang.data_ptr(), ws.data_ptr(), d_img.data_ptr(),
                     dweight[:, e:].data_ptr(), dweight[:, 2 * e:].data_ptr(), ld, n, hw, co, e, _s())
    return d_img


def _ids(ids: torch.Tensor, name: str) -> torch.Tensor:
    if not ids.is_cuda:
        raise ValueError(f"{name}: token ids must be a CUDA tensor (no CPU path), got {ids.device}")
    if ids.dtype not in (torch.int64, torch.int32, torch.int16, torch.uint8, torch.int8):
        raise ValueError(f"{name}: token ids must be an integer tensor, got {ids.dtype}")
    return ids.to(torch.int64).contiguous()


def row_lengths(ids):
    ids = _ids(ids, "row_lengths")
    n, L = ids.shape
    out = torch.empty(n, dtype=torch.int64, device=ids.device)
    lib().row_lengths(ids.data_ptr(), n, L, out.data_ptr(), _s())
    return out


def embedding_fwd(ids, table):
    ids = _ids(ids, "embedding_fwd"); _chk(table, "embedding_fwd table")
    if ids.device != table.device:
        raise ValueError("embedding_fwd: ids and table on different devices")
    v, e = table.shape
    out = torch.empty(tuple(ids.shape) + (e,), dtype=torch.float32, device=table.device)
    lib().embedding_fwd(ids.data_ptr(), table.data_ptr(), out.data_ptr(), ids.numel(), e, v, _s())
    return out


def embedding_bwd(ids, dout, vocab):
    ids = _ids(ids, "embedding_bwd"); _chk(dout, "embedding_bwd dout")
    if ids.device != dout.device or dout.numel() != ids.numel() * dout.shape[-1]:
        raise ValueError("embedding_bwd: dout must be (ids.shape, e) on the ids' device")
    e = dout.shape[-1]
    dt = torch.empty((vocab, e), dtype=torch.float32, device=dout.device)
# ... 534 lines not shown
```

### include/dcnet_hip.h

```cpp
#ifndef DCNET_HIP_H
#define DCNET_HIP_H

#include <stdint.h>

#ifdef __cplusplus
extern "C" {
#endif

#define DCN_OK 0
#define DCN_ERR_ARG (-1)
#define DCN_ERR_LAUNCH (-2)

#define DCN_AMAX_WORDS 64
#define DCN_SLAB_COUNTERS 4096

#define DCN_ACT_NONE 0
#define DCN_ACT_LEAKY 1

#define DCN_ABI_VERSION 313

const char* dcn_last_error(void);
int dcn_version(void);

int dcn_nchw_to_nhwc(const float* src, float* dst, int n, int c, int h, int w, int c_pad, void* stream);
int dcn_nhwc_to_nchw(const float* src, float* dst, int n, int c, int h, int w, int ld, void* stream);
int dcn_oihw_to_ohwi(const float* src, float* dst, int co, int ci, int kh, int kw, int ci_pad, void* stream);
int dcn_ohwi_to_oihw(const float* src, float* dst, int co, int ci, int kh, int kw, int ci_pad, void* stream);

int dcn_conv2d_fwd(const float* x, const float* w, float* y,
                   int n, int h, int wd, int cin, int cout, int ksize, int stride,
                   const float* scale, const float* shift, int act, float slope,
                   const float* residual, int ldr, int ldy,
                   float* stats, int accumulate, const float* f8_scales,
                   const uint32_t* amax_x, const uint32_t* amax_w, uint32_t* amax_y, float* w_split, int w_split_ready,
                   void* stream);
int dcn_absmax(const float* x, int64_t rows, int c, int ld, uint32_t* amax, void* stream);
int dcn_conv2d_stats_rows(int n, int h, int wd, int cout, int ksize, int stride);
int dcn_conv1_tile(int64_t rows, int cout, int ntaps, int cin, int stats, int storage);
int dcn_l2norm_score_fwd_form(int c);
int dcn_bn_apply_form(int c, int params_aligned);
int dcn_igemm_split_build(int kind, int ksteps);
int dcn_gemm3_variant(void);
int dcn_f8_scale(const float* x, int64_t rows, int c, int ld, float* scale, void* ws, void* stream);

int dcn_conv2d_bwd_data(const float* dy, int lddy, const float* w, float* wt, float* dx,
                        int n, int h, int wd, int cin, int cout, int ksize, int stride,
                        int accumulate, const float* f8_scales, const uint32_t* amax_dy, const uint32_t* amax_w,
                        int wt_ready, const float* wt_split, void* stream);
int dcn_conv2d_bwd_data_tap(const float* dy, int lddy, const float* w, float* wt, float* dx,
                            int n, int h, int wd, int cin, int cout, int ksize, int stride,
                            int accumulate, const float* f8_scales, const uint32_t* amax_dy, const uint32_t* amax_w,
                            int wt_ready, const float* wt_split,
                            const float* tap_y, const float* tap_mean, const float* tap_invstd, const float* tap_gamma,
                            const float* tap_beta, int tap_act, float tap_slope, float* tap_stats, int tap_stats_rows,
                            int* tap_rows, void* stream);
int dcn_conv2d_bwd_data_tap_rows(int n, int h, int wd, int cin, int cout, int ksize, int stride);
int dcn_conv2d_pre_supported(int n, int h, int wd, int cin, int cout, int ksize, int stride);
int dcn_conv2d_fwd_pre(const float* x, const float* w, float* y, int n, int h, int wd, int cin, int cout, int ksize, int stride,
                       const float* pre_scale, const float* pre_shift, int pre_act, float pre_slope,
                       int ldy, float* stats, const uint32_t* amax_x, const uint32_t* amax_w, void* stream);
int dcn_conv2d_bwd_weight_pre_supported(int n, int h, int wd, int cin, int cout, int ksize, int stride);
int dcn_conv2d_bwd_weight_pre(const float* x, int ldx, const float* dy, int lddy, float* dw, float* ws, uint32_t* counters,
                              int n, int h, int wd, int cin, int cout, int ksize, int stride,
                              const float* pre_scale, const float* pre_shift, int pre_act, float pre_slope,
                              const uint32_t* amax_x, const uint32_t* amax_dy, void* stream);
int dcn_filter_job_bytes(void);
int dcn_prepare_filters(const void* jobs, int njobs, int total_blocks, int total_amax_blocks,
                        uint32_t* amax_all, int64_t amax_words, void* stream);

int64_t dcn_conv2d_geom_size(int n, int h, int wd, int ksize, int stride);
int dcn_conv2d_geom(uint32_t* table, int n, int h, int wd, int ksize, int stride, void* stream);

int dcn_conv2d_bwd_weight(const float* x, int ldx, const float* dy, int lddy, float* dw, float* ws, uint32_t* counters,
                          const uint32_t* geom,
                          int n, int h, int wd, int cin, int cout, int ksize, int stride,
                          const uint32_t* amax_x, const uint32_t* amax_dy, void* stream);
int64_t dcn_conv2d_bwd_weight_ws(int n, int h, int wd, int cin, int cout, int ksize, int stride);
int dcn_stem_bwd_weight_bn(const float* x, const float* y, const float* dout, int lddo,
                           const float* mean, const float* invstd, const float* gamma, const float* beta,
                           int act, float slope, const float* sums, int64_t count,
                           int n, int h, int wd, int cout, float* dw, float* ws, void* stream);
int64_t dcn_stem_bwd_weight_bn_ws(int n, int h, int wd);
int dcn_stem_bwd_weight_bn_b16(const float* x, const float* y, const void* dout16, int lddo,
                               const float* mean, const float* invstd, const float* gamma, const float* beta,
                               int act, float slope, const float* sums, int64_t count,
                               int n, int h, int wd, int cout, float* dw, float* ws, void* stream);

int dcn_gemm3_supported(int m, int n, int k, int batch);
int dcn_gemm3_presplit(const float* src, int ld, int64_t bs, float* dst, int ldd, int64_t bsd, int batch, int rows, int c,
                       const uint32_t* amax, void* stream);
int dcn_gemm3(const float* a, int lda, int64_t a_bs, int a_t, const float* b, int ldb, int64_t b_bs, int b_t,
              float* c, int ldc, int64_t c_bs, const float* row_scale, int64_t rs_bs,
              int m, int n, int k, int batch, int accumulate, const uint32_t* amax_a, const uint32_t* amax_b, void* stream);

int64_t dcn_bn_ws(int c);
int dcn_bn_finalize(const float* stats, int rows, int c, int64_t count,
                    const float* gamma, const float* beta, float eps, float momentum,
                    float* running_mean, float* running_var,
                    float* mean, float* invstd, float* scale, float* shift, float* ws, void* stream);
int dcn_bn_fold(const float* gamma, const float* beta, const float* running_mean, const float* running_var,
                float eps, int c, float* scale, float* shift, void* stream);
int dcn_channel_stats(const float* x, int64_t rows, int c, int ld, float* stats, void* stream);
int dcn_channel_stats_rows(int64_t rows);
int dcn_scale_act(const float* y, const float* scale, const float* shift, int act, float slope,
                  const float* residual, float* out, int64_t rows, int c, int ldo, uint32_t* amax, void* stream);
int dcn_bn_act_amax_bound(const uint32_t* amax_y, const float* scale, const float* shift, int c, float slope,
                          uint32_t* amax_out, void* stream);
int dcn_bn_act_bwd_reduce(const float* y, const float* dout, int lddo, const float* mean, const float* invstd,
                          const float* gamma, const float* beta, int act, float slope,
                          int64_t rows, int c, float* stats, void* stream);
int dcn_bn_bwd_sums(const float* stats, int rows, int c, float* sums, float* ws, void* stream);
int dcn_bn_act_bwd_apply(const float* y, const float* dout, int lddo, const float* mean, const float* invstd,
                         const float* gamma, const float* beta, int act, float slope,
                         const float* sums, int64_t count, int64_t rows, int c, float* dy, uint32_t* amax, void* stream);
int dcn_act_bwd(const float* out, const float* dout, int lddo, float slope, int64_t rows, int c, float* dy, void* stream);

int64_t dcn_coattn_e_size(int b, int hw);
int64_t dcn_coattn_saved_size(int b, int hw, int c);
int64_t dcn_coattn_fwd_ws(int b, int hw, int c);
int dcn_coattn_fwd(const float* f1, const float* f2, int ldf, int64_t bsf, float* f1_attn, float* f2_attn, int ldo,
                   int64_t bso, float* E, float* rinv, float* cinv, float* ws,
                   int b, int hw, int c, float temperature, void* stream);
int64_t dcn_coattn_bwd_ws(int b, int hw, int c);
int dcn_coattn_bwd(const float* f1, const float* f2, int ldf, int64_t bsf,
                   const float* d_f1_attn, const float* d_f2_attn, int lddo, int64_t bsdo,
                   const float* f1_attn, const float* f2_attn, int ldo, int64_t bso,
                   const float* E, const float* rinv, const float* cinv,
                   float* d_f1, float* d_f2, int lddf, int64_t bsdf, int accumulate, float* ws,
                   int b, int hw, int c, float temperature, void* stream);

int dcn_l2norm_score_fwd(const float* x, int ldx, float* out, int ldo, float* norm,
                         const float* q, float* score, float* score_flip, int64_t rows, int rows_per_image, int c,
                         float out_scale, int accumulate, void* stream);
int dcn_l2norm_score_bwd(const float* out, int ldo, const float* norm, const float* dout, int lddo,
                         const float* q, const float* dscore, const float* dscore_flip, float* dx, int lddx, float* dq,
                         int64_t rows, int rows_per_image, int c, void* stream);
int dcn_rowdot_fwd(const float* x, int ldx, const float* q, int flip, float* score, int64_t rows, int rows_per_image, int c,
                   void* stream);
int dcn_rowdot_bwd(const float* x, int ldx, const float* q, int flip, const float* dscore, float* dx, int lddx, float* dq,
                   int64_t rows, int rows_per_image, int c, void* stream);

int dcn_phrase_attn_fwd(const float* context, const float* embedded, const int64_t* ids,
                        const float* w0, const float* b0, const float* w1, const float* b1,
                        float* attn, float* out, float* vnorm, int n, int l, int d, int e, int normalize, void* stream);
int64_t dcn_phrase_attn_bwd_ws(int n, int d, int heads);
int dcn_phrase_attn_bwd(const float* context, const float* embedded, const float* w0, const float* w1,
                        const float* attn, const float* out, const float* vnorm, const float* dout,
                        float* dcontext, float* dembedded, float* dw, float* ws,
                        int n, int l, int d, int e, int normalize, void* stream);
int dcn_colsum(const float* in, int ld, int rows, int cols, float* out, void* stream);

int dcn_locemb_fwd(const float* coord, const float* w, const float* b, const float* gamma, const float* beta,
                   float* running_mean, float* running_var, float momentum, float eps, int training, int64_t count,
                   int p, float* e8, float* xhat, float* stat, double* mom, void* stream);
int dcn_locemb_bwd(const float* coord, const float* w, const float* gamma, const float* beta, const float* xhat,
                   const float* stat, const float* de_a, const float* de_b, const double* dmom, int training, int p,
                   float* grads, void* stream);
int dcn_head_obj(const float* const* logits, const int* ld, const float* const* sim, const int* hw, const float* e8,
                 float* const* only_obj, float* obj_map, float* objn, float* x, int b, void* stream);
int dcn_pad_rows(const float* src, int lds, float* dst, int ldd, int rows, int cols, int cols_out, void* stream);
int dcn_locbn_fwd(const float* m, const double* mom, const float* bias, const float* gamma, const float* beta,
                  float* running_mean, float* running_var, float momentum, float eps, int training, int batch,
                  int64_t count, int c, float* mp, float* bp, float* saved, void* stream);
int dcn_locbn_bwd(const float* m, const double* mom, const float* bias, const float* gamma, const float* running_mean,
                  const float* saved, const float* dmp, int64_t dmp_bs, const float* dbp, int training, int batch,
                  int64_t count, int c, float* dm, float* out, double* dmom, void* stream);
int dcn_head_final_fwd(const float* const* logits, const int* ld, const float* const* sim, const int* hw,
                       const float* loc_map, float* const* outbox, float* const* loc_score, float* minmax, int b, void* stream);
int dcn_head_dloc(const float* const* logits, const int* ld, const float* const* sim, const int* hw,
                  const float* const* loc_score, const float* const* d_outbox, const float* const* d_loc,
                  const float* minmax, float* dloc_map, int b, void* stream);
int dcn_head_fold(const float* dx, const float* e8, const float* obj_map, int b, int p, int ppad, float* dobj_map,
                  float* de8, void* stream);
int dcn_head_dlogits(const float* const* logits, const int* ld, const float* const* sim, const int* hw,
                     const float* const* loc_score, const float* const* only_obj, const float* const* d_outbox,
                     const float* const* d_only, const float* obj_map, const float* objn, const float* dobj_map,
                     float* const* dlogits, float* const* dsim, int b, void* stream);

int dcn_k9_fwd(const float* cmap, const float* fv, const int64_t* raw_neg, int pairs, int hw, int e, int top_k, int neg_n,
               int64_t* index, int64_t* neg_idx, float* frame, float* corr, float* negf, void* stream);
int dcn_k9_bwd(const int64_t* index, const int64_t* neg_idx, const float* d_frame, const float* d_corr, const float* d_neg,
               int pairs, int hw, int e, int top_k, int neg_n, float* dfv, void* stream);
int dcn_colnorm_fwd(const float* v, int n, int hw, int e, float* vit, float* cnorm, void* stream);
int dcn_colnorm_bwd(const float* vit, const float* cnorm, const float* dq, const float* extra, int n_extra,
                    int n, int hw, int e, float* dv, void* stream);
int dcn_lagnorm_fwd(const float* context, int n, int l, int d, float* lag, float* lnorm, void* stream);
int dcn_crossmap(const float* lag, const float* vit, const float* conv_w, const float* conv_b, int n, int l, int hw, int e,
                 int64_t* cols, float* lvmap, void* stream);
int dcn_k14_gather(const float* lag, const float* vit, const int64_t* cols, const int64_t* neg, int n, int l, int hw, int e,
                   int neg_n, float* lag_pos, float* neg_cross, void* stream);
int dcn_k14_negscatter(const float* d_neg, const int* csr_off, const int* csr_src, int hw, int e, float* extra, void* stream);
int dcn_k14_dlag(const float* lag, const float* lnorm, const int64_t* cols, const float* d_k, int n, int l, int hw, int e,
                 float* dcontext, void* stream);

int dcn_build_target(const float* bbox, const float* anchors, int size, int n, int* target_i, float* target_f, void* stream);
int dcn_target_dense(const int* target_i, const float* target_f, int size, int n, float* const* bbox_list,
                     float* const* center_list, void* stream);
int dcn_dense_loss_fwd(const float* const* outbox, const float* const* sim, const float* const* negsim, const float* const* loc,
                       const int* target_i, const float* target_f, int size, int n, float* vals, float* lse, float* out,
                       void* stream);
int dcn_dense_loss_bwd(const float* const* outbox, const float* const* sim, const float* const* negsim, const float* const* loc,
                       const int* target_i, const float* target_f, const float* lse, const float* grad_out, int size, int n,
                       float* const* d_outbox, float* const* d_sim, float* const* d_negsim, float* const* d_loc, void* stream);
int dcn_contrastive_fwd(const float* q, const float* pos, const float* neg, int64_t rows, int e, int m, float temperature,
                        float* loss_rows, float* loss, void* stream);
int dcn_contrastive_bwd(const float* q, const float* pos, const float* neg, int64_t rows, int e, int m, float temperature,
                        const float* grad_out, float* dq, float* dpos, float* dneg, void* stream);
int dcn_decode_boxes(const float* const* outbox, const float* anchors, int size, int n, float* boxes, int* cellinfo, void* stream);
int dcn_box_iou(const float* box1, const float* box2, int n, float* iou, void* stream);

int dcn_conv2d_stats_rows_b16(int n, int h, int wd, int cout, int ksize, int stride);
int dcn_conv2d_fwd_b16(const void* x, const void* w16, void* y, int y_f32, int n, int h, int wd, int cin, int cout, int ksize, int stride,
                       const float* scale, const float* shift, int act, float slope, const void* residual, int ldr, int ldy,
                       float* stats, int accumulate, void* stream);
int dcn_conv2d_bwd_data_b16(const void* dy, int lddy, const void* wt16, void* dx, int dx_f32, int n, int h, int wd, int cin, int cout,
                            int ksize, int stride, int accumulate, const void* tap_y, const float* tap_mean, const float* tap_invstd,
                            const float* tap_gamma, const float* tap_beta, int tap_act, float tap_slope, float* tap_stats,
                            int tap_stats_rows, int* tap_rows, void* stream);
int64_t dcn_conv2d_bwd_weight_ws_b16(int n, int h, int wd, int cin, int cout, int ksize, int stride);
int dcn_conv2d_bwd_weight_b16(const void* x, int ldx, const void* dy, int lddy, float* dw, float* ws, uint32_t* counters, const uint32_t* geom,
                              int n, int h, int wd, int cin, int cout, int ksize, int stride, void* stream);
int dcn_scale_act_b16(const void* y, int y_f32, const float* scale, const float* shift, int act, float slope, const void* residual,
                      int ldr, void* out, int out_f32, int64_t rows, int c, int ldo, void* stream);
int dcn_bn_act_bwd_reduce_rows_b16(int64_t rows);
int dcn_bn_act_bwd_reduce_b16(const void* y, int y_f32, const void* dout, int dout_f32, int lddo, const float* mean, const float* invstd,
                              const float* gamma, const float* beta, int act, float slope, int64_t rows, int c, float* stats,
                              void* stream);
int dcn_bn_act_bwd_apply_b16(const void* y, int y_f32, const void* dout, int dout_f32, int lddo, const float* mean, const float* invstd,
                             const float* gamma, const float* beta, int act, float slope, const float* sums, int64_t count,
                             int64_t rows, int c, void* dy, void* stream);
int dcn_cast_rows(const void* src, int src_b16, int lds, void* dst, int dst_b16, int ldd, int64_t rows, int c, int accumulate,
                  void* stream);
int dcn_upsample2_nhwc_b16(const void* src, int lds, void* dst, int ldd, int n, int h, int w, int c, void* stream);
int dcn_upsample2_nhwc_bwd_b16(const void* ddst, int ldd, void* dsrc, int lds, int n, int h, int w, int c, int accumulate,
                               void* stream);

int dcn_quant_rows_e4m3(const void* x, int ld, int64_t rows, int c, void* q, int ldq, void* scales, void* stream);
int dcn_quant_job_bytes(void);
int dcn_quant_rows_e4m3_batched(const void* jobs, int njobs, int blocks, int64_t elements, void* stream);
int dcn_quant_fusable(int c);
int dcn_scale_act_b16_q(const void* y, const float* scale, const float* shift, int act, float slope, const void* residual, int ldr, void* out,
                        int64_t rows, int c, void* q8, void* qs, void* stream);
int dcn_bn_act_bwd_apply_b16_q(const void* y, const void* dout, int lddo, const float* mean, const float* invstd, const float* gamma,
                               const float* beta, int act, float slope, const float* sums, int64_t count, int64_t rows, int c, void* dy,
                               void* q8, void* qs, void* stream);
int dcn_conv2d_stats_rows_f8(int n, int h, int wd, int cout, int ksize, int stride);
int dcn_conv2d_fwd_f8(const void* x8, const void* xs, const void* w8, const void* ws, void* y, int y_f32, int n, int h, int wd, int cin, int cout,
                      int ksize, int stride, const float* scale, const float* shift, int act, float slope, const void* residual, int ldr,
                      int ldy, float* stats, int accumulate, void* stream);
int dcn_conv2d_bwd_data_f8(const void* dy8, const void* dys, const void* wt8, const void* wts, void* dx, int dx_f32, int n, int h, int wd, int cin,
                           int cout, int ksize, int stride, int accumulate, const void* tap_y, const float* tap_mean, const float* tap_invstd,
                           const float* tap_gamma, const float* tap_beta, int tap_act, float tap_slope, float* tap_stats, int tap_stats_rows,
                           int* tap_rows, void* stream);

int dcn_post_topk(const float* const* outbox, const float* const* feat, const int64_t* feat_strides, const int* grids,
                  const float* anchors, int size, int n, int e, int top_k, const float* ratio, const float* dw, const float* dh,
                  const int64_t* frame_hw, float* boxes, float* scores, float* feats, int64_t* cells, void* stream);
int dcn_post_fusion(const float* center, const float* ref, const float* ref_score, const unsigned char* valid, int n, int k, int r,
                    int e, float* fused, int64_t* best, void* stream);

int dcn_bank_write(const float* x, int ldx, float* bank, float* split, int64_t rows, int c, void* stream);
int dcn_coattn_bank_fwd(const float* f1, const float* f2, const float* f1s, const float* f2s, int64_t bsf, float* f1_attn,
                        float* f2_attn, int ldo, int64_t bso, float* E, float* rinv, float* cinv, float* ws, int b, int hw, int c,
                        float temperature, void* stream);
int dcn_post_fusion_bank(const float* feats, const float* scores, int n, int k, int r, int e, float* fused, int64_t* best,
                         void* stream);

typedef struct DcnPrepJob {
  int64_t src_off;
  int32_t h, w;
  int32_t rh, rw;
  int32_t top, left;
  int32_t flip;
  int32_t hsv;
  float a_v;
  int32_t warp;
  double minv[6];
} DcnPrepJob;
int64_t dcn_clip_prep_ws(int n, int size);
int dcn_clip_prep(const uint8_t* src, int64_t src_bytes, const DcnPrepJob* jobs, const DcnPrepJob* jobs_host, int n, int size,
                  uint8_t* ws, float* out, uint8_t* u8_out, void* stream);

// ... 75 lines not shown
```

Baseline: 86.82 clips/s.

## Fuse co-attention backward dP products via K-concatenated GEMM and addend epilogue

Adds a co-attention backward path that concatenates [dO1s|f1] and [f2|dO2s] along K, so the two dP products become one GEMM of depth 2C. The dA kernel then reads a single combined gradient matrix instead of two. The passthrough gradient slice is now added in the GEMM epilogue instead of a separate copy kernel. L2Norm writes straight into the left half of a 2C buffer for scales above 0, which drops the copy_slice in the forward. The cost is extra workspace, new amax slots and a stricter layout contract on the input buffer.

New measurement: 87.30 clips/s, median of 6. No clear change (+0.6%).

```diff
diff --git a/dcnet_amd/csrc/coattn.hip b/dcnet_amd/csrc/coattn.hip
--- a/dcnet_amd/csrc/coattn.hip
+++ b/dcnet_amd/csrc/coattn.hip
@@ -72,7 +72,7 @@
   cinv[(size_t)bb * hw + j] = 1.f / s;
 }
 
-enum { AM_ONE = 0, AM_DO1, AM_DO2, AM_DO1S, AM_DO2S, AM_DA, AM_DP1, AM_DP2, AM_SLOTS };
+enum { AM_ONE = 0, AM_DO1, AM_DO2, AM_DO1S, AM_DO2S, AM_DA, AM_DP1, AM_DP2, AM_DOS, AM_DEL1, AM_DEL2, AM_G, AM_SLOTS };
 __global__ __launch_bounds__(256) void amax_init_kernel(unsigned* __restrict__ w) {
   for (int i = threadIdx.x; i < AM_SLOTS * DCN_AMAX_WORDS; i += 256) w[i] = i < DCN_AMAX_WORDS ? 0x3F800000u : 0u;
 }
@@ -80,33 +80,39 @@
 __global__ __launch_bounds__(256) void rowdot_scale_kernel(const float* __restrict__ d, int ldd, int64_t bsd,
                                                            const float* __restrict__ o, int ldo, int64_t bso, int hw,
                                                            const float* __restrict__ inv, int64_t rows, int c,
-                                                           float* __restrict__ delta, float* __restrict__ ds,
-                                                           unsigned* __restrict__ amax_d, unsigned* __restrict__ amax_ds) {
+                                                           float* __restrict__ delta, float* __restrict__ ds, int ldds,
+                                                           unsigned* __restrict__ amax_d, unsigned* __restrict__ amax_ds,
+                                                           unsigned* __restrict__ amax_delta) {
   __shared__ float red[4];
   const int lane = threadIdx.x & 63;
   const int64_t row = (int64_t)blockIdx.x * 4 + (threadIdx.x >> 6);
-  float vmax = 0.f, s = 0.f;
+  float vmax = 0.f, s = 0.f, acc = 0.f;
   if (row < rows) {
     const int64_t bb = row / hw, i = row - bb * hw;
     s = inv[row];
-    float acc = 0.f;
     for (int k = lane * 4; k < c; k += 256) {
       const f32x4 dv = *reinterpret_cast<const f32x4*>(d + bb * bsd + i * ldd + k);
       const f32x4 ov = *reinterpret_cast<const f32x4*>(o + bb * bso + i * ldo + k);
       acc += dv[0] * ov[0] + dv[1] * ov[1] + dv[2] * ov[2] + dv[3] * ov[3];
-      *reinterpret_cast<f32x4*>(ds + row * c + k) = dv * s;
+      *reinterpret_cast<f32x4*>(ds + row * ldds + k) = dv * s;
       vmax = fmaxf(fmaxf(vmax, fmaxf(fabsf(dv[0]), fabsf(dv[1]))), fmaxf(fabsf(dv[2]), fabsf(dv[3])));
     }
     acc = wave_sum(acc);
     if (lane == 0) delta[row] = acc;
   }
   const float vs = wave_max(vmax * s);
-  amax_update_block(amax_d, vmax, red);
-  __syncthreads();
+  if (amax_d) {
+    amax_update_block(amax_d, vmax, red);
+    __syncthreads();
+  }
   amax_update_block(amax_ds, vs, red);
-}
-
-template <bool ESPLIT, bool OSPLIT = false>
+  if (amax_delta) {
+    __syncthreads();
+    amax_update_block(amax_delta, fabsf(acc), red);
+  }
+}
+
+template <bool ESPLIT, bool OSPLIT = false, bool KCAT = false>
 __global__ __launch_bounds__(256) void dA_kernel(const float* __restrict__ E, float* __restrict__ dP1, const float* __restrict__ dP2,
                                                  const float* __restrict__ rinv, const float* __restrict__ cinv,
                                                  const float* __restrict__ d1, const float* __restrict__ d2,
@@ -135,13 +141,17 @@
       e = *reinterpret_cast<const f32x4*>(E + row * ldE + j);
     }
     const f32x4 p1 = *reinterpret_cast<const f32x4*>(dP1 + row * ldE + j);
-    const f32x4 p2 = *reinterpret_cast<const f32x4*>(dP2 + row * ldE + j);
+    f32x4 p2 = {0.f, 0.f, 0.f, 0.f};
+    if constexpr (!KCAT) p2 = *reinterpret_cast<const f32x4*>(dP2 + row * ldE + j);
     const float ri = rinv[row], di = d1[row];
     f32x4 o;
 #pragma unroll
     for (int k = 0; k < 4; ++k) {
       float v = 0.f;
-      if (j + k < hw) v = t * e[k] * ((p1[k] - di) * ri + (p2[k] - d2[bb * hw + j + k]) * cinv[bb * hw + j + k]);
+      if (j + k < hw) {
+        if constexpr (KCAT) v = t * e[k] * ((p1[k] - di * ri) - d2[bb * hw + j + k] * cinv[bb * hw + j + k]);
+        else v = t * e[k] * ((p1[k] - di) * ri + (p2[k] - d2[bb * hw + j + k]) * cinv[bb * hw + j + k]);
+      }
       o[k] = v;
     }
     if constexpr (OSPLIT) {
@@ -163,6 +173,11 @@
 __global__ __launch_bounds__(64) void da_bound_kernel(const unsigned* __restrict__ a1, const unsigned* __restrict__ a2, float t,
                                                       unsigned* __restrict__ out) {
   const float b = 2.f * t * (__uint_as_float(amax_read(a1)) + __uint_as_float(amax_read(a2)));
+  out[threadIdx.x & (DCN_AMAX_WORDS - 1)] = __float_as_uint(b);
+}
+__global__ __launch_bounds__(64) void da_bound_cat_kernel(const unsigned* __restrict__ ag, const unsigned* __restrict__ ad1,
+                                                          const unsigned* __restrict__ ad2, float t, unsigned* __restrict__ out) {
+  const float b = t * (__uint_as_float(amax_read(ag)) + __uint_as_float(amax_read(ad1)) + __uint_as_float(amax_read(ad2)));
   out[threadIdx.x & (DCN_AMAX_WORDS - 1)] = __float_as_uint(b);
 }
 
@@ -269,21 +284,91 @@
   return rc;
 }
 
+static bool on_kcat(int b, int hw, int c) { return !gemm3_two_product_bwd() && on_gemm3(b, hw, c); }
+
 extern "C" int64_t dcn_coattn_bwd_ws(int b, int hw, int c) {
-  return (int64_t)2 * b * hw * ld_pad(hw) + (int64_t)2 * b * hw * c + (int64_t)2 * b * hw + AM_SLOTS * DCN_AMAX_WORDS +
-         (on_gemm3(b, hw, c) ? (int64_t)2 * b * hw * c + 4 : 0);
-}
-
-extern "C" int dcn_coattn_bwd(const float* f1, const float* f2, int ldf, int64_t bsf,
-                              const float* d_f1_attn, const float* d_f2_attn, int lddo, int64_t bsdo,
-                              const float* f1_attn, const float* f2_attn, int ldo, int64_t bso,
-                              const float* E, const float* rinv, const float* cinv,
-                              float* d_f1, float* d_f2, int lddf, int64_t bsdf, int accumulate, float* ws,
-                              int b, int hw, int c, float temperature, void* stream_) {
+  const int64_t rows = (int64_t)b * hw;
+  return 2 * rows * ld_pad(hw) + 2 * rows * c + 2 * rows + AM_SLOTS * DCN_AMAX_WORDS + (on_gemm3(b, hw, c) ? 2 * rows * c + 4 : 0);
+}
+extern "C" int64_t dcn_coattn_bwd_add_ws(int b, int hw, int c) {
+  const int64_t rows = (int64_t)b * hw;
+  if (on_kcat(b, hw, c))
+    return rows * ld_pad(hw) + 4 * rows * c + 2 * rows + AM_SLOTS * DCN_AMAX_WORDS;
+  return dcn_coattn_bwd_ws(b, hw, c);
+}
+
+namespace {
+
+__global__ __launch_bounds__(256) void addend_copy_kernel(const float* __restrict__ a, int lda, int64_t bsa, float* __restrict__ d, int ldd,
+                                                          int64_t bsd, int hw, int c, int64_t total4) {
+  const int c4 = c >> 2;
+  for (int64_t i = (int64_t)blockIdx.x * 256 + threadIdx.x; i < total4; i += (int64_t)gridDim.x * 256) {
+    const int64_t row = i / c4; const int k = (int)(i - row * c4) * 4;
+    const int64_t bb = row / hw, r = row - bb * hw;
+    *reinterpret_cast<f32x4*>(d + bb * bsd + r * ldd + k) = *reinterpret_cast<const f32x4*>(a + bb * bsa + r * lda + k);
+  }
+}
+
+int coattn_bwd_kcat(const float* f1, const float* f2, int ldf, int64_t bsf, const float* d_f1_attn, const float* d_f2_attn, int lddo,
+                    int64_t bsdo, const float* f1_attn, const float* f2_attn, int ldo, int64_t bso, const float* E, const float* rinv,
+                    const float* cinv, float* d_f1, float* d_f2, int lddf, int64_t bsdf, int accumulate, const float* add1,
+                    const float* add2, int ldadd, int64_t bsadd, float* ws, int b, int hw, int c, float temperature, hipStream_t stream) {
+  const int ldE = ld_pad(hw), c2 = 2 * c;
+  const long long rows = (long long)b * hw, bsE = (long long)hw * ldE, bsc = (long long)hw * c2;
+  float* G = ws;
+  float* Acat = G + rows * ldE;
+  float* Bcat = Acat + rows * c2;
+  float* dO1s = Acat; float* dO2s = Bcat + c;
+  float* del1 = Bcat + rows * c2;
+  float* del2 = del1 + rows;
+  unsigned* am = reinterpret_cast<unsigned*>(del2 + rows);
+  hipLaunchKernelGGL(amax_init_kernel, dim3(1), dim3(256), 0, stream, am);
+  DCN_CHECK_LAUNCH("coattn amax_init");
+  auto slot = [&](int i) { return am + i * DCN_AMAX_WORDS; };
+  hipLaunchKernelGGL(rowdot_scale_kernel, dim3(cdiv(rows, 4)), dim3(256), 0, stream, d_f1_attn, lddo, bsdo, f1_attn, ldo, bso, hw, rinv, rows, c, del1, dO1s,
+                     c2, (unsigned*)nullptr, slot(AM_DOS), slot(AM_DEL1));
+  DCN_CHECK_LAUNCH("rowdot_scale");
+  hipLaunchKernelGGL(rowdot_scale_kernel, dim3(cdiv(rows, 4)), dim3(256), 0, stream, d_f2_attn, lddo, bsdo, f2_attn, ldo, bso, hw, cinv, rows, c, del2, dO2s,
+                     c2, (unsigned*)nullptr, slot(AM_DOS), slot(AM_DEL2));
+  DCN_CHECK_LAUNCH("rowdot_scale");
+  int rc;
+  if ((rc = gemm3_presplit(dO1s, c2, bsc, dO1s, c2, bsc, b, hw, c, slot(AM_DOS), stream))) return rc;
+  if ((rc = gemm3_presplit(dO2s, c2, bsc, dO2s, c2, bsc, b, hw, c, slot(AM_DOS), stream))) return rc;
+  if ((rc = gemm3_presplit(f1, ldf, bsf, Acat + c, c2, bsc, b, hw, c, slot(AM_ONE), stream))) return rc;
+  if ((rc = gemm3_presplit(f2, ldf, bsf, Bcat, c2, bsc, b, hw, c, slot(AM_ONE), stream))) return rc;
+  const float* f1s = E + dcn_coattn_e_size(b, hw);
+  const float* f2s = f1s + rows * c;
+  const long long bss = (long long)hw * c;
+  if ((rc = gemm3_launch(Acat, c2, bsc, 0, Bcat, c2, bsc, 0, G, ldE, bsE, nullptr, 0, hw, hw, c2, b, 0, slot(AM_DOS), slot(AM_ONE), stream, slot(AM_G)))) return rc;
+  hipLaunchKernelGGL(da_bound_cat_kernel, dim3(1), dim3(64), 0, stream, slot(AM_G), slot(AM_DEL1), slot(AM_DEL2), temperature, slot(AM_DA));
+  DCN_CHECK_LAUNCH("dA bound");
+  const int64_t total4 = rows * (ldE / 4);
+  int64_t g = (total4 + 255) / 256; if (g > 1024) g = 1024;
+  const int pid_da = prof_begin(31, (double)total4 * 16.0 * 3.0, stream);
+  hipLaunchKernelGGL((dA_kernel<true, true, true>), dim3((int)g), dim3(256), 0, stream, E, G, (const float*)nullptr, rinv, cinv, del1, del2, hw, ldE, temperature,
+                     total4, slot(AM_DA));
+  prof_end(pid_da, stream);
+  DCN_CHECK_LAUNCH("dA");
+  if ((rc = gemm3_launch(G, ldE, bsE, 0, f2s, c, bss, 1, d_f1, lddf, bsdf, nullptr, 0, hw, c, hw, b, accumulate, slot(AM_DA), slot(AM_ONE), stream, nullptr, add1, ldadd, bsadd))) return rc;
+  if ((rc = gemm3_launch(E, ldE, bsE, 0, dO2s, c2, bsc, 1, d_f1, lddf, bsdf, nullptr, 0, hw, c, hw, b, 1, slot(AM_ONE), slot(AM_DOS), stream))) return rc;
+  if ((rc = gemm3_launch(G, ldE, bsE, 1, f1s, c, bss, 1, d_f2, lddf, bsdf, nullptr, 0, hw, c, hw, b, accumulate, slot(AM_DA), slot(AM_ONE), stream, nullptr, add2, ldadd, bsadd))) return rc;
+  return gemm3_launch(E, ldE, bsE, 1, dO1s, c2, bsc, 1, d_f2, lddf, bsdf, nullptr, 0, hw, c, hw, b, 1, slot(AM_ONE), slot(AM_DOS), stream);
+}
+
+}
+
+static int coattn_bwd_impl(const float* f1, const float* f2, int ldf, int64_t bsf,
+                           const float* d_f1_attn, const float* d_f2_attn, int lddo, int64_t bsdo,
+                           const float* f1_attn, const float* f2_attn, int ldo, int64_t bso,
+                           const float* E, const float* rinv, const float* cinv,
+                           float* d_f1, float* d_f2, int lddf, int64_t bsdf, int accumulate,
+                           const float* add1, const float* add2, int ldadd, int64_t bsadd, float* ws,
+                           int b, int hw, int c, float temperature, void* stream_, bool kcat) {
   hipStream_t stream = (hipStream_t)stream_;
   DCN_CHECK_ARG(f1 && f2 && d_f1_attn && d_f2_attn && f1_attn && f2_attn && E && rinv && cinv && d_f1 && d_f2 && ws,
                 "coattn_bwd: null pointer");
   DCN_CHECK_ARG(b > 0 && hw > 0 && c > 0 && c % 32 == 0, "coattn_bwd: bad shape");
+  DCN_CHECK_ARG(!add1 == !add2, "coattn_bwd: one addend without the other");
   if (ldf <= 0) ldf = c;
   if (ldo <= 0) ldo = c;
   if (lddo <= 0) lddo = c;
@@ -292,6 +377,24 @@
   if (bso <= 0) bso = (int64_t)hw * ldo;
   if (bsdo <= 0) bsdo = (int64_t)hw * lddo;
   if (bsdf <= 0) bsdf = (int64_t)hw * lddf;
+  if (add1) {
+    if (ldadd <= 0) ldadd = c;
+    if (bsadd <= 0) bsadd = (int64_t)hw * ldadd;
+    DCN_CHECK_ARG(ldadd % 4 == 0 && bsadd % 4 == 0 && lddf % 4 == 0 && bsdf % 4 == 0 && (((uintptr_t)add1 | (uintptr_t)add2 | (uintptr_t)d_f1 | (uintptr_t)d_f2) & 15) == 0,
+                  "coattn_bwd: addend / gradient rows must be 16-byte aligned");
+  }
+  if (kcat && on_kcat(b, hw, c))
+    return coattn_bwd_kcat(f1, f2, ldf, bsf, d_f1_attn, d_f2_attn, lddo, bsdo, f1_attn, f2_attn, ldo, bso, E, rinv, cinv, d_f1, d_f2, lddf, bsdf,
+                           accumulate, add1, add2, ldadd, bsadd, ws, b, hw, c, temperature, stream);
+  if (add1) {
+    const int64_t total4 = (int64_t)b * hw * (c / 4);
+    int64_t ga = (total4 + 255) / 256; if (ga > 8192) ga = 8192;
+    hipLaunchKernelGGL(addend_copy_kernel, dim3((int)ga), dim3(256), 0, stream, add1, ldadd, bsadd, d_f1, lddf, bsdf, hw, c, total4);
+    DCN_CHECK_LAUNCH("coattn addend");
+    hipLaunchKernelGGL(addend_copy_kernel, dim3((int)ga), dim3(256), 0, stream, add2, ldadd, bsadd, d_f2, lddf, bsdf, hw, c, total4);
+    DCN_CHECK_LAUNCH("coattn addend");
+    accumulate = 1;
+  }
   const int ldE = ld_pad(hw);
   const long long rows = (long long)b * hw;
   float* dP1 = ws;
@@ -305,10 +408,10 @@
   DCN_CHECK_LAUNCH("coattn amax_init");
   auto slot = [&](int i) { return am + i * DCN_AMAX_WORDS; };
   hipLaunchKernelGGL(rowdot_scale_kernel, dim3(cdiv(rows, 4)), dim3(256), 0, stream, d_f1_attn, lddo, bsdo, f1_attn, ldo, bso, hw, rinv, rows, c, del1, dO1s,
-                     slot(AM_DO1), slot(AM_DO1S));
+                     c, slot(AM_DO1), slot(AM_DO1S), (unsigned*)nullptr);
   DCN_CHECK_LAUNCH("rowdot_scale");
   hipLaunchKernelGGL(rowdot_scale_kernel, dim3(cdiv(rows, 4)), dim3(256), 0, stream, d_f2_attn, lddo, bsdo, f2_attn, ldo, bso, hw, cinv, rows, c, del2, dO2s,
-                     slot(AM_DO2), slot(AM_DO2S));
+                     c, slot(AM_DO2), slot(AM_DO2S), (unsigned*)nullptr);
   DCN_CHECK_LAUNCH("rowdot_scale");
   const int64_t total4 = rows * (ldE / 4);
   int64_t g = (total4 + 255) / 256; if (g > 8192) g = 8192;
@@ -362,3 +465,24 @@
   return tn_gemm_batched(E, ldE, (long long)hw * ldE, dO1s, c, (long long)hw * c, d_f2, lddf, bsdf,
                          nullptr, hw, ldE, c, hw, b, 1, stream, slot(AM_ONE), slot(AM_DO1S));
 }
+
+extern "C" int dcn_coattn_bwd(const float* f1, const float* f2, int ldf, int64_t bsf,
+                              const float* d_f1_attn, const float* d_f2_attn, int lddo, int64_t bsdo,
+                              const float* f1_attn, const float* f2_attn, int ldo, int64_t bso,
+                              const float* E, const float* rinv, const float* cinv,
+                              float* d_f1, float* d_f2, int lddf, int64_t bsdf, int accumulate, float* ws,
+                              int b, int hw, int c, float temperature, void* stream) {
+  return coattn_bwd_impl(f1, f2, ldf, bsf, d_f1_attn, d_f2_attn, lddo, bsdo, f1_attn, f2_attn, ldo, bso, E, rinv, cinv, d_f1, d_f2, lddf, bsdf,
+                         accumulate, nullptr, nullptr, 0, 0, ws, b, hw, c, temperature, stream, false);
+}
+
+extern "C" int dcn_coattn_bwd_add(const float* f1, const float* f2, int ldf, int64_t bsf,
+                                  const float* d_f1_attn, const float* d_f2_attn, int lddo, int64_t bsdo,
+                                  const float* f1_attn, const float* f2_attn, int ldo, int64_t bso,
+                                  const float* E, const float* rinv, const float* cinv,
+                                  float* d_f1, float* d_f2, int lddf, int64_t bsdf, int accumulate,
+                                  const float* add1, const float* add2, int ldadd, int64_t bsadd, float* ws,
+                                  int b, int hw, int c, float temperature, void* stream) {
+  return coattn_bwd_impl(f1, f2, ldf, bsf, d_f1_attn, d_f2_attn, lddo, bsdo, f1_attn, f2_attn, ldo, bso, E, rinv, cinv, d_f1, d_f2, lddf, bsdf,
+                         accumulate, add1, add2, ldadd, bsadd, ws, b, hw, c, temperature, stream, true);
+}
diff --git a/dcnet_amd/csrc/gemm3.hip b/dcnet_amd/csrc/gemm3.hip
--- a/dcnet_amd/csrc/gemm3.hip
+++ b/dcnet_amd/csrc/gemm3.hip
@@ -35,6 +35,7 @@
   int tiles_m, tiles_n;
   const float* row_scale; long long rs_bs;
   int accumulate;
+  const float* addend; long long add_bs; int ldadd;
   const unsigned* amax_a; const unsigned* amax_b;
   unsigned* amax_out;
   int var;
@@ -228,6 +229,7 @@
 
   const float dq = 1.f / (g3_pow2_scale(amax_read(p.amax_a)) * g3_pow2_scale(amax_read(p.amax_b)));
   float* __restrict__ cb = p.C + batch * p.c_bs;
+  const float* ab = p.addend ? p.addend + batch * p.add_bs : nullptr;
   const float* rs = p.row_scale ? p.row_scale + batch * p.rs_bs : nullptr;
   float vmax = 0.f;
 #pragma unroll
@@ -243,7 +245,8 @@
         if (n >= p.N) continue;
         float v = acc[mi][ni][r] * f;
         float* dst = cb + (long long)m * p.ldc + n;
-        if (p.accumulate) v += *dst;
+        if (ab) v += ab[(long long)m * p.ldadd + n];
+        else if (p.accumulate) v += *dst;
         *dst = v;
         vmax = fmaxf(vmax, fabsf(v));
       }
@@ -274,7 +277,7 @@
   }
 }
 
-DCN_KNOB(g_gemm3, "Gemm3", 1, "gemm3.hip: the co-attention products on pre-split operands (0 = implicit-GEMM / weight-gradient tiles; + 256 * v = schedule variant v; + 16 * bits = timing ablations, results WRONG)",
+DCN_KNOB(g_gemm3, "Gemm3", 1, "gemm3.hip: the co-attention products on pre-split operands (0 = implicit-GEMM / weight-gradient tiles; + 256 * v = schedule variant v; + 16 * bits = timing ablations, results WRONG; + 2: dcn_coattn_bwd_add on the two-product backward)",
          nullptr, "-DG3_ABL=1", G3_ABL != 0, [](int v) { return (v & 0xF0) != 0; });
 DCN_KNOB(g_gemm3_h1, "H1gemm3", 1, "gemm3.hip: one f16 piece per operand in the bf16 precision modes (0 = both pieces, fp32-accurate co-attention)");
 
@@ -297,6 +300,7 @@
 
 int gemm3_variant() { const int v = g_gemm3 >> 8; return (v == 1 || v == 2) ? v : 0; }
 extern "C" int dcn_gemm3_variant() { return gemm3_variant(); }
+bool gemm3_two_product_bwd() { return (g_gemm3 & 2) != 0; }
 
 bool gemm3_applicable(int M, int N, int K, int batch) {
   return g_gemm3 && (igemm_precision() == 4 || igemm_precision() == 2) && M >= 512 && N >= 256 && K >= 64 && batch >= 1;
@@ -315,7 +319,7 @@
 int gemm3_launch(const float* A, int lda, long long a_bs, int at, const float* B, int ldb, long long b_bs, int bt,
                  float* C, int ldc, long long c_bs, const float* row_scale, long long rs_bs,
                  int M, int N, int K, int batch, int accumulate, const unsigned* amax_a, const unsigned* amax_b, hipStream_t stream,
-                 unsigned* amax_out) {
+                 unsigned* amax_out, const float* addend, int ldadd, long long add_bs) {
   DCN_CHECK_ARG(A && B && C && amax_a && amax_b, "gemm3: null pointer");
   DCN_CHECK_ARG(lda % 4 == 0 && ldb % 4 == 0 && a_bs % 4 == 0 && b_bs % 4 == 0 && (((uintptr_t)A | (uintptr_t)B) & 15) == 0, "gemm3: 16-byte rows");
   G3Params p{};
@@ -326,7 +330,7 @@
   p.a_cols = at ? (M + 7) / 8 * 8 : k16; p.b_cols = bt ? (N + 7) / 8 * 8 : k16;
   DCN_CHECK_ARG(p.a_cols <= lda && p.b_cols <= ldb, "gemm3: rows shorter than the tile reads (lda=%d ldb=%d)", lda, ldb);
   p.tiles_m = cdiv(M, G3_BM); p.tiles_n = cdiv(N, G3_BN);
-  p.row_scale = row_scale; p.rs_bs = rs_bs; p.accumulate = accumulate; p.amax_a = amax_a; p.amax_b = amax_b; p.amax_out = amax_out; p.abl = (g_gemm3 >> 4) & 15; p.var = gemm3_variant();
+  p.row_scale = row_scale; p.rs_bs = rs_bs; p.accumulate = accumulate; p.addend = addend; p.ldadd = ldadd; p.add_bs = add_bs; p.amax_a = amax_a; p.amax_b = amax_b; p.amax_out = amax_out; p.abl = (g_gemm3 >> 4) & 15; p.var = gemm3_variant();
   const int grid = p.tiles_m * p.tiles_n * batch;
   const int pid = prof_begin(40, 2.0 * batch * (double)M * N * K, stream);
   int rc;
diff --git a/dcnet_amd/csrc/igemm.h b/dcnet_amd/csrc/igemm.h
--- a/dcnet_amd/csrc/igemm.h
+++ b/dcnet_amd/csrc/igemm.h
@@ -80,12 +80,13 @@
 int dgrad2_launch(const float* dy, int lddy, const float* wt, float* dx, int n, int h, int wd, int cin, int accumulate,
                   const uint32_t* amax_dy, const uint32_t* amax_w, const DcnBnTap* tap, hipStream_t stream);
 bool gemm3_applicable(int M, int N, int K, int batch);
+bool gemm3_two_product_bwd();
 int gemm3_presplit(const float* src, int ld, long long bs, float* dst, int ldd, long long bsd, int batch, int rows, int c,
                    const unsigned* amax, hipStream_t stream);
 int gemm3_launch(const float* A, int lda, long long a_bs, int at, const float* B, int ldb, long long b_bs, int bt,
                  float* C, int ldc, long long c_bs, const float* row_scale, long long rs_bs,
                  int M, int N, int K, int batch, int accumulate, const unsigned* amax_a, const unsigned* amax_b, hipStream_t stream,
-                 unsigned* amax_out = nullptr);
+                 unsigned* amax_out = nullptr, const float* addend = nullptr, int ldadd = 0, long long add_bs = 0);
 int igemm_precision();
 extern int g_abl;
 extern int g_wsplit;
diff --git a/dcnet_amd/functions.py b/dcnet_amd/functions.py
--- a/dcnet_amd/functions.py
+++ b/dcnet_amd/functions.py
@@ -134,8 +134,11 @@
 class L2Norm(torch.autograd.Function):
 
     @staticmethod
-    def forward(ctx, x):
-        out, norm, _, _ = ops.l2norm_score_fwd(x)
+    def forward(ctx, x, cat_room: bool = False):
+        out = None
+        if cat_room:
+            out = torch.empty((*x.shape[:-1], 2 * x.shape[-1]), dtype=torch.float32, device=x.device)[..., :x.shape[-1]]
+        out, norm, _, _ = ops.l2norm_score_fwd(x, out=out)
         ctx.save_for_backward(out, norm)
         return out
 
@@ -143,7 +146,7 @@
     def backward(ctx, dout):
         out, norm = ctx.saved_tensors
         dx, _ = ops.l2norm_score_bwd(out, norm, dout.contiguous(), None, None, 0)
-        return dx
+        return dx, None
 
 
 class NormScore(torch.autograd.Function):
@@ -454,12 +457,20 @@
 class CoAttentionPairs(torch.autograd.Function):
 
     @staticmethod
-    def forward(ctx, fv, temperature: float):
+    def forward(ctx, fv, temperature: float, in_cat: bool = False):
         n, h, w, c = fv.shape
         hw = h * w
-        cat = torch.empty((n, hw, 2 * c), dtype=torch.float32, device=fv.device)
-        f = fv.view(n, hw, c)
-        ops.copy_slice(f, cat[..., :c])
+        if in_cat:
+            st = fv.untyped_storage()
+            if (fv.dtype != torch.float32 or fv.stride() != (hw * 2 * c, w * 2 * c, 2 * c, 1) or fv.storage_offset() != 0 or
+                    st.nbytes() != n * hw * 2 * c * 4):
+                raise ValueError("CoAttentionPairs(in_cat=True): fv must be the left half of its own (N,H,W,2C) fp32 buffer")
+            cat = torch.empty(0, dtype=torch.float32, device=fv.device).set_(st, 0, (n, hw, 2 * c), (hw * 2 * c, 2 * c, 1))
+            f = fv.view(n, hw, c)
+        else:
+            cat = torch.empty((n, hw, 2 * c), dtype=torch.float32, device=fv.device)
+            f = fv.view(n, hw, c)
+            ops.copy_slice(f, cat[..., :c])
         E, rc = ops.coattn_fwd(f[0::2], f[1::2], cat[0::2, :, c:], cat[1::2, :, c:], temperature)
         out = cat.view(n, h, w, 2 * c)
         ctx.save_for_backward(fv, out, E, rc)
@@ -474,10 +485,9 @@
         f, cat = fv.view(n, hw, c), out.view(n, hw, 2 * c)
         dcat = dcat.contiguous().view(n, hw, 2 * c)
         df = torch.empty((n, hw, c), dtype=torch.float32, device=f.device)
-        ops.copy_slice(dcat[..., :c], df)
-        ops.coattn_bwd(f[0::2], f[1::2], dcat[0::2, :, c:], dcat[1::2, :, c:], cat[0::2, :, c:], cat[1::2, :, c:],
-                       E, rc, df[0::2], df[1::2], True, ctx.temperature)
-        return df.view(n, h, w, c), None
+        ops.coattn_bwd_add(f[0::2], f[1::2], dcat[0::2, :, c:], dcat[1::2, :, c:], cat[0::2, :, c:], cat[1::2, :, c:],
+                           E, rc, df[0::2], df[1::2], False, ctx.temperature, add1=dcat[0::2, :, :c], add2=dcat[1::2, :, :c])
+        return df.view(n, h, w, c), None, None
 
 
 class CoAttentionCenter(torch.autograd.Function):
diff --git a/dcnet_amd/lib.py b/dcnet_amd/lib.py
--- a/dcnet_amd/lib.py
+++ b/dcnet_amd/lib.py
@@ -61,6 +61,8 @@
     "dcn_coattn_fwd": (I, [P, P, I, L, P, P, I, L, P, P, P, P, I, I, I, F, P]),
     "dcn_coattn_bwd_ws": (L, [I, I, I]),
     "dcn_coattn_bwd": (I, [P, P, I, L, P, P, I, L, P, P, I, L, P, P, P, P, P, I, L, I, P, I, I, I, F, P]),
+    "dcn_coattn_bwd_add_ws": (L, [I, I, I]),
+    "dcn_coattn_bwd_add": (I, [P, P, I, L, P, P, I, L, P, P, I, L, P, P, P, P, P, I, L, I, P, P, I, L, P, I, I, I, F, P]),
     "dcn_l2norm_score_fwd": (I, [P, I, P, I, P, P, P, P, L, I, I, F, I, P]),
     "dcn_l2norm_score_bwd": (I, [P, I, P, P, I, P, P, P, P, I, P, L, I, I, P]),
     "dcn_rowdot_fwd": (I, [P, I, P, I, P, L, I, I, P]),
@@ -168,7 +170,7 @@
                 "dcn_conv2d_bwd_weight_pre_supported", "dcn_gemm3_supported", "dcn_channel_stats_rows", "dcn_filter_job_bytes", "dcn_prof_records",
                 "dcn_conv2d_stats_rows_b16", "dcn_bn_act_bwd_reduce_rows_b16", "dcn_conv2d_stats_rows_f8", "dcn_quant_fusable", "dcn_quant_job_bytes",
                 "dcn_conv1_tile", "dcn_l2norm_score_fwd_form", "dcn_bn_apply_form", "dcn_igemm_split_build", "dcn_gemm3_variant"}
-ABI_VERSION = 313
+ABI_VERSION = 314
 
 
 class DcnError(RuntimeError):
diff --git a/dcnet_amd/model.py b/dcnet_amd/model.py
--- a/dcnet_amd/model.py
+++ b/dcnet_amd/model.py
@@ -297,10 +297,11 @@
 
     def _scale_pairs(self, s: int, raw_s, flang, flang_attn):
         ops.region("mapping")
-        fv = L2Norm.apply(self.mapping_visu[s](raw_s, self.visumodel._tap_amax[s]))
+        in_cat = s > 0
+        fv = L2Norm.apply(self.mapping_visu[s](raw_s, self.visumodel._tap_amax[s]), in_cat)
         ops.region("corr")
         one = ops.amax_const(raw_s.device, 1.0) if ops.use_amax() else None
-        corr_raw = self.corr_conv[s][0](CoAttentionPairs.apply(fv, self.temperature), one)
+        corr_raw = self.corr_conv[s][0](CoAttentionPairs.apply(fv, self.temperature, in_cat), one)
         corr, sim, neg_sim = NormScore.apply(corr_raw, flang_attn, self.training)
         return fv, corr, sim, neg_sim, self._fusion_head(s, corr, flang)
 
diff --git a/dcnet_amd/ops.py b/dcnet_amd/ops.py
--- a/dcnet_amd/ops.py
+++ b/dcnet_amd/ops.py
@@ -937,6 +937,24 @@
                      b, hw, c, float(temperature), _s())
 
 
+def coattn_bwd_add(f1, f2, d_out1, d_out2, out1, out2, E, rc, d_f1, d_f2, accumulate, temperature, add1=None, add2=None):
+    b, hw, c = f1.shape
+    ws = scratch(lib().coattn_bwd_add_ws(b, hw, c), f1.device, slot=0)
+    assert f1.stride() == f2.stride() and d_out1.stride() == d_out2.stride() and out1.stride() == out2.stride()
+    assert d_f1.stride() == d_f2.stride()
+    if (add1 is None) != (add2 is None):
+        raise ValueError("coattn_bwd_add: add1 and add2 come together")
+    if add1 is not None and (add1.stride() != add2.stride() or add1.stride(2) != 1 or add1.shape != f1.shape or add2.shape != f1.shape):
+        raise ValueError("coattn_bwd_add: add1 / add2 must be (b, hw, c) views with equal strides and a contiguous last dimension")
+    lib().coattn_bwd_add(f1.data_ptr(), f2.data_ptr(), f1.stride(1), f1.stride(0),
+                         d_out1.data_ptr(), d_out2.data_ptr(), d_out1.stride(1), d_out1.stride(0),
+                         out1.data_ptr(), out2.data_ptr(), out1.stride(1), out1.stride(0),
+                         E.data_ptr(), rc[0].data_ptr(), rc[1].data_ptr(),
+                         d_f1.data_ptr(), d_f2.data_ptr(), d_f1.stride(1), d_f1.stride(0), int(accumulate),
+                         _p(add1), _p(add2), add1.stride(1) if add1 is not None else 0, add1.stride(0) if add1 is not None else 0,
+                         ws.data_ptr(), b, hw, c, float(temperature), _s())
+
+
 def gemm3_presplit(x, amax, out=None):
     b, rows, c = x.shape
     if out is None:
diff --git a/include/dcnet_hip.h b/include/dcnet_hip.h
--- a/include/dcnet_hip.h
+++ b/include/dcnet_hip.h
@@ -17,7 +17,7 @@
 #define DCN_ACT_NONE 0
 #define DCN_ACT_LEAKY 1
 
-#define DCN_ABI_VERSION 313
+#define DCN_ABI_VERSION 314
 
 const char* dcn_last_error(void);
 int dcn_version(void);
@@ -128,6 +128,14 @@
                    const float* E, const float* rinv, const float* cinv,
                    float* d_f1, float* d_f2, int lddf, int64_t bsdf, int accumulate, float* ws,
                    int b, int hw, int c, float temperature, void* stream);
+int64_t dcn_coattn_bwd_add_ws(int b, int hw, int c);
+int dcn_coattn_bwd_add(const float* f1, const float* f2, int ldf, int64_t bsf,
+                       const float* d_f1_attn, const float* d_f2_attn, int lddo, int64_t bsdo,
+                       const float* f1_attn, const float* f2_attn, int ldo, int64_t bso,
+                       const float* E, const float* rinv, const float* cinv,
+                       float* d_f1, float* d_f2, int lddf, int64_t bsdf, int accumulate,
+                       const float* add1, const float* add2, int ldadd, int64_t bsadd, float* ws,
+                       int b, int hw, int c, float temperature, void* stream);
 
 int dcn_l2norm_score_fwd(const float* x, int ldx, float* out, int ldo, float* norm,
                          const float* q, float* score, float* score_flip, int64_t rows, int rows_per_image, int c,
```
